# folbricht/desync

Hardware: AMD Instinct MI355X
Metric: GiB/s chunked (device-resident blob→cut list), 16/64/256KiB, 1/2/4/8 MI355X (higher is better)
Workload: dtype u8; 1 GPU; 32 GiB uniform blob per GPU (BASELINE config 5 shard shape), desync make min/avg/max 16/64/256 KiB, device-resident blob -> cut list in HBM; bytes_per_gpu=34359738368, chunks=524384, parallelism=single GPU, jobs_in_flight=4

## Files before the change

### desync_amd/_lib.py

```python
from __future__ import annotations

import ctypes
import os
import threading

HERE = os.path.dirname(os.path.abspath(__file__))
LIB_PATH = os.environ.get("DSX_LIB_PATH") or os.path.join(HERE, "libdsx.so")

DSX_OUT_HOST = 0
DSX_OUT_DEVICE = 1
DSX_NO_SYNC = 2
DSX_TIMED = 16
DSX_SEAM_MAX_CANDS = 1024
DSX_SEAM_MAX_CUTS = 1024

DSX_OK = 0
DSX_E_MIN_TOO_SMALL = -1
DSX_E_MIN_GT_MAX = -2
DSX_E_MIN_GT_AVG = -3
DSX_E_AVG_GT_MAX = -4
DSX_E_AVG_RANGE = -5
DSX_E_INVAL = -6
DSX_E_CAPACITY = -7
DSX_E_HIP = -8
DSX_E_NOMEM = -9
DSX_E_INTERRUPTED = -10
DSX_E_IO = -11
DSX_E_STATE = -12
DSX_E_INTERNAL = -13
DSX_E_RESYNC = -14
DSX_E_PEER = -15
DSX_STREAM_EOF = 1
DSX_STREAM_SYNC = 2
DSX_SEAM_DEVICE = 8
DSX_SEAM_LAST = 1
DSX_SEAM_REWALKED = 2
DSX_SEAM_ERROR = 4
DSX_SEAM_REDO = 16

EXPORTS = (
    "dsx_params_init", "dsx_strerror", "dsx_abi_version", "dsx_ctx_create", "dsx_ctx_destroy",
    "dsx_last_error", "dsx_cancel", "dsx_cut_device", "dsx_sync", "dsx_result", "dsx_cut_host",
    "dsx_cut_fd", "dsx_stream_begin", "dsx_stream_push", "dsx_stream_pop", "dsx_stream_advance",
    "dsx_stream_done", "dsx_stream_end", "dsx_stream_chunk_data", "dsx_stream_buffer",
    "dsx_stream_commit", "dsx_stream_flush", "dsx_stream_ids", "dsx_stream_chunk_id",
    "dsx_stream_pop_many", "dsx_stream_window", "dsx_stream_unpop", "dsx_shard_local", "dsx_shard_resolve",
    "dsx_selftest_boundary", "dsx_gen_uniform", "dsx_gen_dedup", "dsx_chunk_ids",
    "dsx_get_stats", "dsx_debug_trace", "dsx_index_fd", "dsx_index_host", "dsx_copy",
    "dsx_ids_fd", "dsx_ids_host", "dsx_progress", "dsx_shard_resolve_async", "dsx_shard_collect",
    "dsx_ctx_stream", "dsx_stamps_begin", "dsx_stamps_end", "dsx_host_copy",
    "dsx_host_sha512_256", "dsx_idset_create", "dsx_idset_destroy", "dsx_idset_count", "dsx_dedup",
)
DSX_DIGEST_SHA512_256 = 0
DSX_DIGEST_SHA256 = 1
DSX_ENDS_DEVICE = 4
DSX_HOST_SHA_SCALAR = 1
DSX_IDS_DEVICE = 32
DSX_SIZES = 64
DSX_POS_NONE = 0xFFFFFFFF


class Params(ctypes.Structure):

    _fields_ = [
        ("min", ctypes.c_uint64), ("avg", ctypes.c_uint64), ("max", ctypes.c_uint64),
        ("discriminator", ctypes.c_uint32), ("inverse_odd", ctypes.c_uint32),
        ("qmax", ctypes.c_uint32), ("qbias", ctypes.c_uint32), ("rot", ctypes.c_int32),
        ("reserved", ctypes.c_uint32),
    ]


class Stats(ctypes.Structure):
    _fields_ = [
        ("chunks", ctypes.c_uint64), ("candidates", ctypes.c_uint64), ("pieces", ctypes.c_uint64),
        ("repaired_segments", ctypes.c_uint64), ("dense_fallbacks", ctypes.c_uint64),
        ("scan_ms", ctypes.c_float), ("stitch_ms", ctypes.c_float),
        ("chunks_discarded", ctypes.c_uint64),
        ("device_bytes", ctypes.c_uint64),
        ("host_tail_chunks", ctypes.c_uint64),
    ]


class DedupTotals(ctypes.Structure):

    _fields_ = [(n, ctypes.c_uint64) for n in
                ("total", "unique", "in_seed", "size", "size_not_in_seed")]


class ScanStamp(ctypes.Structure):

    _fields_ = [(n, ctypes.c_uint64) for n in
                ("seq", "bytes", "t_first", "t_last", "wave_cycles", "wave_ticks", "waves", "reserved")]

    @property
    def ms(self):
        return (self.t_last - self.t_first) / 1e5

    @property
    def mhz(self):
        return 100.0 * self.wave_cycles / self.wave_ticks if self.wave_ticks else 0.0

    @property
    def busy(self):
        span = self.t_last - self.t_first
        return self.wave_ticks / (self.waves * span) if self.waves and span else 0.0


class Seam(ctypes.Structure):
    _fields_ = [
        ("shard_start", ctypes.c_uint64), ("shard_len", ctypes.c_uint64), ("total", ctypes.c_uint64),
        ("first_cand_beyond", ctypes.c_uint64), ("exit_cut", ctypes.c_uint64),
        ("window_end", ctypes.c_uint64), ("entry", ctypes.c_uint64),
        ("ncands", ctypes.c_uint32), ("ncuts", ctypes.c_uint32),
        ("flags", ctypes.c_uint32), ("pad", ctypes.c_uint32),
        ("cands", ctypes.c_uint64 * DSX_SEAM_MAX_CANDS),
        ("cuts", ctypes.c_uint64 * DSX_SEAM_MAX_CUTS),
    ]


_lib = None
_lock = threading.RLock()


def _share_torch_hip_runtime():
    try:
        import torch
    except ImportError:
        return
    path = os.path.join(os.path.dirname(torch.__file__), "lib", "libamdhip64.so")
    if os.path.exists(path):
        ctypes.CDLL(path, mode=ctypes.RTLD_GLOBAL)


PRODUCT_ENV = ("DSX_TAIL_SPLIT", "DSX_LANE_TARGET", "DSX_SEG_FLOOR", "DSX_SCAN_NT",
               "DSX_DIGEST_PC", "DSX_DIGEST_LPT", "DSX_INDEX_WINDOW", "DSX_INDEX_SLOT",
               "DSX_INDEX_READERS", "DSX_INDEX_HOST_TAIL", "DSX_HOST_THREADS")
DIAG_ENV = {"DSX_SCAN_VARIANT": "0", "DSX_SCAN_CFG": "0", "DSX_FUSE": "0", "DSX_TEST_MODE": None,
            "DSX_DIGEST_PC_CHUNKS": "2", "DSX_PREFETCH": "0", "DSX_REGIONS_PER_SLOT": "1",
            "DSX_SCAN_LINE": "1", "DSX_SCAN_TRACE": "0", "DSX_WAVE_MAJOR": "1",
            "DSX_FIXUP_FAST": "1", "DSX_FINISH": "1", "DSX_SEG_MAX": "4", "DSX_SEG_TARGET": "4096",
            "DSX_DIGEST_PF": "1", "DSX_TAIL_MULT": "1", "DSX_LANE_BYTES": None,
            "DSX_STITCH_CUS": "0", "DSX_SCAN_MASK": "0", "DSX_SCAN_PRIO": None,
            "DSX_STREAM_BATCH": None, "DSX_NOOP_BEFORE_SCAN": None, "DSX_WALK_WGS": "2",
            "DSX_WALK_NT": "576", "DSX_TAIL_LOG": None, "DSX_FEED_THREADS": None, "DSX_FEED_MULTI": None,
            "DSX_FEED_MID": None, "DSX_SIDE_PRIO": "1",
            "DSX_FEED_CUT_END": None, "DSX_SHARE_NS": "45", "DSX_SHARE_PC": "1", "DSX_SHARE_SLACK": "0", "DSX_CTX_PRIO": "1", "DSX_FEED_EXTRA": None, "DSX_SHARE_MULTI": "1", "DSX_FINE_TAIL": "33554432", "DSX_FINE_DIV": "4"}


def lib():
    global _lib
    with _lock:
        if _lib is not None:
            return _lib
        if not os.path.exists(LIB_PATH):
            raise ImportError(
                f"{LIB_PATH} is missing: build it with __graft_entry__.build() "
                "(make -C desync_amd/csrc). desync_amd has no CPU fallback.")
        diag_env = [k for k, dflt in DIAG_ENV.items() if os.environ.get(k, "") not in ("", dflt)]
        if diag_env and not os.path.basename(LIB_PATH).startswith("libdsx_diag"):
            raise ImportError(
                f"{', '.join(diag_env)} selects a diagnostic path (scan ablations, other "
                "geometries, rejected experiments), which only the diagnostic build reads: "
                "make -C desync_amd/csrc diag and set "
                "DSX_LIB_PATH=desync_amd/libdsx_diag.so")
        _share_torch_hip_runtime()
        L = ctypes.CDLL(LIB_PATH)
        u64, u32, i32, vp = ctypes.c_uint64, ctypes.c_uint32, ctypes.c_int, ctypes.c_void_p
        P = ctypes.POINTER
        sig = {
            "dsx_params_init": (i32, [u64, u64, u64, P(Params)]),
            "dsx_strerror": (ctypes.c_char_p, [i32]),
            "dsx_abi_version": (i32, []),
            "dsx_ctx_create": (i32, [i32, P(vp)]),
            "dsx_ctx_destroy": (i32, [vp]),
            "dsx_last_error": (ctypes.c_char_p, [vp]),
            "dsx_cancel": (i32, [vp]),
            "dsx_progress": (i32, [vp, P(u64)]),
            "dsx_cut_device": (i32, [vp, vp, u64, P(Params), vp, u64, P(u64), u32]),
            "dsx_sync": (i32, [vp]),
            "dsx_result": (i32, [vp, P(u64)]),
            "dsx_cut_host": (i32, [vp, vp, u64, P(Params), vp, u64, P(u64)]),
            "dsx_cut_fd": (i32, [vp, i32, u64, u64, P(Params), vp, u64, P(u64)]),
            "dsx_stream_begin": (i32, [vp, P(Params)]),
            "dsx_stream_push": (i32, [vp, vp, u64, i32]),
            "dsx_stream_pop": (i32, [vp, P(u64), P(u64)]),
            "dsx_stream_advance": (i32, [vp, u64]),
            "dsx_stream_done": (i32, [vp]),
            "dsx_stream_end": (i32, [vp]),
            "dsx_stream_buffer": (i32, [vp, u64, P(vp)]),
            "dsx_stream_commit": (i32, [vp, u64, i32]),
            "dsx_stream_flush": (i32, [vp, P(u64), P(u64)]),
            "dsx_stream_ids": (i32, [vp, i32]),
            "dsx_stream_chunk_id": (vp, [vp]),
            "dsx_stream_pop_many": (i32, [vp, vp, vp, u64, P(u64), P(u64)]),
            "dsx_stream_window": (i32, [vp, P(vp), P(u64), P(u64)]),
            "dsx_stream_unpop": (i32, [vp, u64]),
            "dsx_stream_chunk_data": (vp, [vp]),
            "dsx_shard_local": (i32, [vp, vp, u64, u64, u64, u64, P(Params), vp, u32]),
            "dsx_shard_resolve": (i32, [vp, vp, i32, i32, vp, vp, u64, P(u64), u32]),
            "dsx_shard_resolve_async": (i32, [vp, vp, i32, i32, vp, u64, vp]),
            "dsx_shard_collect": (i32, [vp, vp, vp, P(ctypes.c_int32), P(u64)]),
            "dsx_ctx_stream": (i32, [vp, P(vp)]),
            "dsx_selftest_boundary": (i32, [vp, P(Params), i32, u64, u64, P(u64)]),
            "dsx_gen_uniform": (i32, [vp, vp, u64, u64, u64]),
            "dsx_gen_dedup": (i32, [vp, vp, u64, u64, u64, ctypes.c_double]),
            "dsx_chunk_ids": (i32, [vp, vp, u64, u64, vp, u64, vp, u32, i32]),
            "dsx_get_stats": (i32, [vp, P(Stats)]),
            "dsx_copy": (i32, [vp, vp, vp, u64]),
            "dsx_index_fd": (i32, [vp, i32, u64, u64, P(Params), i32, vp, vp, u64, P(u64)]),
            "dsx_index_host": (i32, [vp, vp, u64, P(Params), i32, vp, vp, u64, P(u64)]),
            "dsx_debug_trace": (i32, [vp, vp, u64, P(u64), P(u64)]),
            "dsx_ids_fd": (i32, [vp, i32, u64, u64, u64, vp, u64, i32, vp]),
            "dsx_ids_host": (i32, [vp, vp, u64, u64, vp, u64, i32, vp]),
            "dsx_stamps_begin": (i32, [vp, u64]),
            "dsx_stamps_end": (i32, [vp, vp, u64, P(u64)]),
            "dsx_host_copy": (i32, [vp, vp, u64, i32]),
            "dsx_host_sha512_256": (i32, [vp, vp, u64, vp, i32, i32]),
            "dsx_idset_create": (i32, [vp, vp, u64, u32, P(vp)]),
            "dsx_idset_destroy": (i32, [vp, vp]),
            "dsx_idset_count": (i32, [vp, P(u64), P(u64)]),
            "dsx_dedup": (i32, [vp, vp, vp, u64, u64, vp, vp, vp, P(DedupTotals), u32]),
        }
        for name, (res, args) in sig.items():
            f = getattr(L, name)
            f.restype = res
            f.argtypes = args
        _lib = L
        return L


class DsxError(RuntimeError):
    def __init__(self, code, detail=""):
        self.code = code
        msg = lib().dsx_strerror(code).decode()
        super().__init__(f"{msg}" + (f": {detail}" if detail else ""))


def check(rc, ctx=None):
    if rc < 0:
        detail = ""
        if ctx is not None and rc in (DSX_E_HIP, DSX_E_INTERNAL, DSX_E_NOMEM):
            d = lib().dsx_last_error(ctx)
            detail = d.decode() if d else ""
        raise DsxError(rc, detail)
    return rc


class Context:

    def __init__(self, device=0):
        h = ctypes.c_void_p()
        rc = lib().dsx_ctx_create(int(device), ctypes.byref(h))
        if rc != DSX_OK:
            why = lib().dsx_last_error(None)
            raise DsxError(rc, f"cannot create a dsx context on HIP device {device}"
                           + (f" ({why.decode()})" if why else ""))
        self.h = h
        self.device = device

    def close(self):
        if self.h:
            lib().dsx_ctx_destroy(self.h)
            self.h = None

    def __del__(self):
        try:
            self.close()
        except Exception:
            pass

    def stats(self):
        s = Stats()
        check(lib().dsx_get_stats(self.h, ctypes.byref(s)), self.h)
        return s

    def stamps_begin(self, max_launches):
        check(lib().dsx_stamps_begin(self.h, int(max_launches)), self.h)
        self._stamp_cap = int(max_launches)

    def stamps_end(self):
        cap = getattr(self, "_stamp_cap", 0)
        buf = (ScanStamp * max(1, cap))()
        n = ctypes.c_uint64()
        check(lib().dsx_stamps_end(self.h, buf, cap, ctypes.byref(n)), self.h)
        return list(buf[:min(cap, n.value)])


_default = {}
_pool = {}


def default_context(device=0):
    ctx = _default.get(device)
    if ctx is None:
        ctx = Context(device)
        _default[device] = ctx
    return ctx


_POOL_IDLE = 4


def _env_key(device):
    return (device, tuple(sorted((k, v) for k, v in os.environ.items() if k.startswith("DSX_"))))


def acquire_context(device=0):
    key = _env_key(device)
    ctx = None
    with _lock:
        stale = [c for k in list(_pool) if k[0] == device and k != key for c in _pool.pop(k)]
        idle = _pool.setdefault(key, [])
        while idle and ctx is None:
            ctx = idle.pop()
            ctx = ctx if ctx.h else None
    for c in stale:
        c.close()
    if ctx is None:
        ctx = Context(device)
        ctx._pool_key = key
    return ctx


def release_context(ctx):
    if ctx is None or not ctx.h:
        return
    key = getattr(ctx, "_pool_key", None) or _env_key(ctx.device)
    with _lock:
        idle = _pool.setdefault(key, [])
        if len(idle) < _POOL_IDLE:
            idle.append(ctx)
            return
    ctx.close()


class pooled_context:

    def __init__(self, device=0):
        self.device = device
        self.ctx = None

    def __enter__(self):
        self.ctx = acquire_context(self.device)
        return self.ctx

    def __exit__(self, *exc):
        release_context(self.ctx)
        self.ctx = None
        return False


def reset_context_pool():
    with _lock:
        idle = [c for cs in _pool.values() for c in cs]
        _pool.clear()
    for c in idle:
        c.close()
```

### desync_amd/csrc/dsx_api.cpp

```cpp
#include <hip/hip_runtime.h>
#include <unistd.h>

#include <algorithm>
#include <atomic>
#include <cerrno>
#include <cmath>
#include <cstdarg>
#include <cstdio>
#include <cstdlib>
#include <cstring>
#include <deque>
#include <string>
#include <vector>

#include "dsx_engine.h"

using namespace dsx;

static_assert(sizeof(dsx_seam_t) == 7 * 8 + 4 * 4 + 8 * (DSX_SEAM_MAX_CANDS + DSX_SEAM_MAX_CUTS),
              "dsx_seam_t layout");

static void release_kept(dsx_ctx* c);


int set_hip_err(dsx_ctx* c, hipError_t e, const char* what) {
  char buf[256];
  snprintf(buf, sizeof buf, "%s: %s", what, hipGetErrorString(e));
  c->err = buf;
  return e == hipErrorOutOfMemory || e == hipErrorMemoryAllocation ? DSX_E_NOMEM : DSX_E_HIP;
}

static uint32_t discriminator_from_avg(uint64_t avg) {
  volatile double a = (double)avg;
  volatile double den = -1.42888852e-7 * a;
  den = den + 1.33237515;
  volatile double q = a / den;
  if (!(q >= 1.0 && q < 4294967296.0)) return 0u;
  return (uint32_t)q;
}

static uint32_t mod_inverse32(uint32_t d) {
  uint32_t x = d;
  for (int i = 0; i < 5; ++i) x *= 2u - d * x;
  return x;
}

extern "C" int dsx_abi_version(void) { return DSX_ABI_VERSION; }

extern "C" int dsx_params_init(uint64_t min, uint64_t avg, uint64_t max, dsx_params_t* out) {
  if (!out) return DSX_E_INVAL;
  if (min < 48) return DSX_E_MIN_TOO_SMALL;
  if (min > max) return DSX_E_MIN_GT_MAX;
  if (min > avg) return DSX_E_MIN_GT_AVG;
  if (avg > max) return DSX_E_AVG_GT_MAX;
  const uint32_t d = discriminator_from_avg(avg);
  if (d == 0) return DSX_E_AVG_RANGE;
  const uint32_t k = (uint32_t)__builtin_ctz(d);
  const uint32_t odd = d >> k;
  memset(out, 0, sizeof *out);
  out->min = min;
  out->avg = avg;
  out->max = max;
  out->discriminator = d;
  out->inverse_odd = mod_inverse32(odd);
  out->qbias = odd > 1u ? 1u : 0u;
  out->qmax = 0xFFFFFFFFu / d - out->qbias;
  out->rot = (int32_t)k;
  return DSX_OK;
}

extern "C" const char* dsx_strerror(int code) {
  switch (code) {
    case DSX_OK: return "ok";
    case DSX_E_MIN_TOO_SMALL: return "min chunk size too small, must be over 48";
    case DSX_E_MIN_GT_MAX: return "min chunk size must not be greater than max";
    case DSX_E_MIN_GT_AVG: return "min chunk size must not be greater than avg";
    case DSX_E_AVG_GT_MAX: return "avg chunk size must not be greater than max";
    case DSX_E_AVG_RANGE: return "avg chunk size out of range for discriminatorFromAvg";
    case DSX_E_INVAL: return "invalid argument";
    case DSX_E_CAPACITY: return "output capacity too small";
    case DSX_E_HIP: return "HIP runtime error";
    case DSX_E_NOMEM: return "out of memory";
    case DSX_E_INTERRUPTED: return "interrupted";
    case DSX_E_IO: return "I/O error";
    case DSX_E_STATE: return "invalid stream state";
    case DSX_E_INTERNAL: return "internal error";
    case DSX_E_RESYNC: return "seam records changed: all-gather them again and resolve again";
    case DSX_E_PEER: return "another rank failed (its seam record carries DSX_SEAM_ERROR)";
    default: return "unknown error";
  }
}

static TestConsts make_tc(const dsx_params_t* p) {
  TestConsts tc;
  tc.d = p->discriminator;
  tc.dm1 = p->discriminator - 1u;
  tc.inv = p->inverse_odd;
  tc.qmax = p->qmax;
  tc.qbias = p->qbias;
  tc.rot = (uint32_t)p->rot;
  tc.rcp = 1.0f / (float)p->discriminator;
  tc.c0 = 12582911.0f;
  tc.madc = p->discriminator - 1u - (p->discriminator << 22);
  const uint32_t k = (uint32_t)p->rot;
  tc.tadd = p->inverse_odd - 1u;
  tc.vmax = (uint32_t)(((1ull << 32) / p->discriminator) << k);
  tc.dodd = p->discriminator >> k;
  tc.ninv = 0u - p->inverse_odd;
  tc.vmax1 = tc.vmax + 1u;
  return tc;
}

static int pick_mode(const dsx_ctx* c, uint32_t d) {
  if (c->force_mode >= 0 && c->force_mode <= 2) {
    if (c->force_mode != 2 || (d & (d - 1u)) != 0) return c->force_mode;
  }
  if ((d & (d - 1u)) != 0) return 2;
  return (d > 1024u && d < (1u << 22)) ? 1 : 0;
}

static char g_create_err[256];

extern "C" int dsx_ctx_create(int device, dsx_ctx_t** out) {
  if (!out) return DSX_E_INVAL;
  *out = nullptr;
  g_create_err[0] = 0;
  dsx_ctx* c = new dsx_ctx();
  c->device = device;
#define CREATE_STEP(expr)                                                              \
  do {                                                                                 \
    hipError_t e_ = (expr);                                                            \
    if (e_ != hipSuccess) {                                                            \
      snprintf(g_create_err, sizeof g_create_err, "%s: %s (%d)", #expr,                \
               hipGetErrorString(e_), (int)e_);                                        \
      dsx_ctx_destroy(c);                                                              \
      return e_ == hipErrorOutOfMemory ? DSX_E_NOMEM : DSX_E_HIP;                      \
    }                                                                                  \
  } while (0)
  CREATE_STEP(hipSetDevice(device));
  hipDeviceProp_t prop;
  CREATE_STEP(hipGetDeviceProperties(&prop, device));
  c->ncu = prop.multiProcessorCount;
  if (const char* v = getenv("DSX_TAIL_SPLIT")) c->tail_split = std::max(0, std::min(8, atoi(v)));
  if (const char* v = getenv("DSX_LANE_TARGET"))
    c->lane_target = (uint32_t)std::max(384, std::min((int)kLineLaneMax, atoi(v)));
  if (const char* v = getenv("DSX_SEG_FLOOR")) c->seg_floor = (uint64_t)std::max(0L, atol(v));
  if (const char* v = getenv("DSX_SCAN_NT")) c->scan_nt = atoi(v) & 3;
  if (const char* v = getenv("DSX_DIGEST_PC")) c->digest_pc = atoi(v);
  if (const char* v = getenv("DSX_DIGEST_LPT")) c->digest_lpt = atoi(v) != 0;
  if (const char* v = getenv("DSX_INDEX_WINDOW")) c->index_window = (uint64_t)std::max(1L << 16, atol(v));
  if (const char* v = getenv("DSX_INDEX_SLOT")) c->index_slot = (uint64_t)std::max(1L << 12, atol(v));
  if (const char* v = getenv("DSX_INDEX_READERS")) c->index_readers = std::max(1, std::min(32, atoi(v)));
  if (const char* v = getenv("DSX_INDEX_HOST_TAIL")) c->index_host_tail = std::max(-1L, atol(v));
#if DSX_DIAG
  if (const char* m = getenv("DSX_TEST_MODE")) c->force_mode = atoi(m);
  if (const char* v = getenv("DSX_SCAN_VARIANT")) c->variant = atoi(v);
  if (const char* v = getenv("DSX_SCAN_CFG")) c->scan_cfg = std::min(5, std::max(0, atoi(v)));
  if (const char* v = getenv("DSX_DIGEST_PC_CHUNKS")) c->digest_pc_chunks = std::max(1, atoi(v));
  if (const char* v = getenv("DSX_PREFETCH")) c->prefetch_batches = std::max(0, atoi(v));
  if (const char* v = getenv("DSX_REGIONS_PER_SLOT")) c->regions_per_slot = std::max(1, atoi(v));
  if (const char* v = getenv("DSX_SCAN_LINE")) c->scan_line = atoi(v) != 0;
  if (const char* v = getenv("DSX_SCAN_TRACE")) {
    c->scan_trace = atoi(v) != 0;
    c->trace_keep = atoi(v) == 2;
  }
  if (const char* v = getenv("DSX_WAVE_MAJOR")) c->wave_major = atoi(v) != 0;
  if (const char* v = getenv("DSX_FIXUP_FAST")) c->fixup_fast = atoi(v) != 0;
  if (const char* v = getenv("DSX_FINISH")) c->finish = atoi(v) != 0;
  if (const char* v = getenv("DSX_FUSE")) c->fuse = atoi(v) != 0;
  if (const char* v = getenv("DSX_SEG_MAX")) c->seg_max_mult = std::max(1, atoi(v));
  if (const char* v = getenv("DSX_SEG_TARGET")) c->seg_target = (uint64_t)std::max(0L, atol(v));
  if (const char* v = getenv("DSX_WALK_WGS")) c->walk_wgs = std::max(1, std::min(4, atoi(v)));
  if (const char* v = getenv("DSX_WALK_NT")) c->walk_nt = atoi(v) == 576 ? 576 : 256;
  if (const char* v = getenv("DSX_DIGEST_PF")) c->digest_pf = atoi(v) != 0;
  if (const char* v = getenv("DSX_TAIL_MULT")) c->tail_mult = std::max(1, std::min(4, atoi(v)));
  if (const char* v = getenv("DSX_LANE_BYTES")) {
    const long lb = atol(v);
    if (lb >= 48 && lb % 48 == 0 && lb <= (long)kMaxLaneBytes) c->lane_bytes_override = (uint32_t)lb;
  }
  if (const char* v = getenv("DSX_STITCH_CUS")) c->stitch_cus = std::max(0, std::min(c->ncu / 2, atoi(v)));
  if (const char* v = getenv("DSX_SCAN_MASK")) c->scan_mask = atoi(v) != 0;
#endif
  {
    int least = 0, greatest = 0;
    CREATE_STEP(hipDeviceGetStreamPriorityRange(&least, &greatest));
#if DSX_DIAG
    if (const char* v = getenv("DSX_CTX_PRIO"))
      if (atoi(v) == 0) greatest = 0;
#endif
    CREATE_STEP(hipStreamCreateWithPriority(&c->stream, hipStreamNonBlocking, greatest));
    CREATE_STEP(hipStreamCreateWithPriority(&c->copy_stream, hipStreamNonBlocking, greatest));
  }
  c->scan_stream = c->stream;
#if DSX_DIAG
  if (c->stitch_cus > 0) {
    hipStream_t ss = nullptr;
    if (c->scan_mask) {
      std::vector<uint32_t> mask((c->ncu + 31) / 32, 0u);
      for (int i = 0; i < c->ncu - c->stitch_cus; ++i) mask[i / 32] |= 1u << (i % 32);
      CREATE_STEP(hipExtStreamCreateWithCUMask(&ss, (uint32_t)mask.size(), mask.data()));
    } else {
      int least = 0, greatest = 0;
      CREATE_STEP(hipDeviceGetStreamPriorityRange(&least, &greatest));
      const char* pv = getenv("DSX_SCAN_PRIO");
      CREATE_STEP(hipStreamCreateWithPriority(&ss, hipStreamNonBlocking,
                                              pv && atoi(pv) == 0 ? least : greatest));
    }
    c->scan_stream = ss;
    for (int i = 0; i < 2; ++i) {
      CREATE_STEP(hipEventCreateWithFlags(&c->ev_scan[i], hipEventDisableTiming));
      CREATE_STEP(hipEventCreateWithFlags(&c->ev_stitch[i], hipEventDisableTiming));
    }
  }
#endif
  CREATE_STEP(hipHostMalloc((void**)&c->h_state, sizeof(HostState), hipHostMallocCoherent));
  CREATE_STEP(hipHostMalloc((void**)&c->h_ring, kQueueDepth * sizeof(HostState), hipHostMallocCoherent));
  memset(c->h_ring, 0, kQueueDepth * sizeof(HostState));
  c->h_cur = c->h_state;
  for (uint32_t i = 0; i < kQueueDepth; ++i)
    CREATE_STEP(hipEventCreateWithFlags(&c->q_ev[i], hipEventDisableTiming));
  CREATE_STEP(hipHostMalloc((void**)&c->h_res, 4 * sizeof(uint64_t)));
#if DSX_DIAG
  CREATE_STEP(hipHostMalloc((void**)&c->h_tasks, dsx_ctx::kTaskRing * sizeof(TaskArgs), hipHostMallocCoherent));
#endif
  memset(c->h_state, 0, sizeof(HostState));
  CREATE_STEP(c->state.ensure(1));
  CREATE_STEP(c->overflow.ensure(kQueueWords));
  CREATE_STEP(hipMemset(c->overflow.p, 0, kQueueWords * sizeof(uint32_t)));
  CREATE_STEP(hipMemset(c->state.p, 0, sizeof(DevState)));
#undef CREATE_STEP
  *out = c;
  return DSX_OK;
}

extern "C" int dsx_ctx_destroy(dsx_ctx_t* c) {
  if (!c) return DSX_OK;
  (void)hipSetDevice(c->device);
  if (c->stream) (void)hipStreamSynchronize(c->stream);
  if (c->copy_stream) (void)hipStreamSynchronize(c->copy_stream);
  if (c->scan_stream && c->scan_stream != c->stream) (void)hipStreamSynchronize(c->scan_stream);
  c->region_cnt.release(); c->region_list.release(); c->overflow.release(); c->rep_cnt.release(); c->rep_from.release();
  c->region_cnt2.release(); c->region_list2.release();
  c->flag_list.release(); c->lane_slot.release(); c->seg_info.release(); c->stage.release();
  c->dg_ends.release(); c->dg_ids.release(); c->dg_queue.release();
  c->dg_order.release(); c->dg_cls.release();
  c->rep.release(); c->out_off.release(); c->out.release(); c->state.release();
  c->seg_info2.release(); c->stage2.release(); c->spec.release(); c->spec2.release();
  release_kept(c);
  c->zero_word.release();
  c->d_seam.release(); c->d_all.release(); c->d_ext.release(); c->d_info.release(); c->d_emit.release();
  if (c->h_res) (void)hipHostFree(c->h_res);
  if (c->h_tasks) (void)hipHostFree(c->h_tasks);
  index_release(c);
  stream_release(c);
  idset_release(c);
  if (c->h_state) (void)hipHostFree(c->h_state);
  if (c->h_ring) (void)hipHostFree(c->h_ring);
  for (uint32_t i = 0; i < kQueueDepth; ++i)
    if (c->q_ev[i]) (void)hipEventDestroy(c->q_ev[i]);
  for (hipEvent_t e : c->pev) (void)hipEventDestroy(e);
  for (auto& v : c->q_pev)
    for (hipEvent_t e : v) (void)hipEventDestroy(e);
  for (int i = 0; i < 2; ++i) {
    if (c->ev_scan[i]) (void)hipEventDestroy(c->ev_scan[i]);
    if (c->ev_stitch[i]) (void)hipEventDestroy(c->ev_stitch[i]);
  }
  if (c->scan_stream && c->scan_stream != c->stream) (void)hipStreamDestroy(c->scan_stream);
  if (c->stream) (void)hipStreamDestroy(c->stream);
  if (c->copy_stream) (void)hipStreamDestroy(c->copy_stream);
  delete c;
  return DSX_OK;
}

extern "C" const char* dsx_last_error(dsx_ctx_t* c) { return c ? c->err.c_str() : g_create_err; }

extern "C" int dsx_cancel(dsx_ctx_t* c) {
  if (!c) return DSX_E_INVAL;
  c->cancel.store(1);
  return DSX_OK;
}

extern "C" int dsx_progress(dsx_ctx_t* c, uint64_t* bytes) {
  if (!c || !bytes) return DSX_E_INVAL;
  uint64_t v = c->prog_done.load();
  if (c->prog_active.load()) {
    const uint64_t cur = ((volatile HostState*)c->h_state)->carry;
    if (cur > v && cur <= c->prog_len.load()) {
      uint64_t seen = v;
      while (seen < cur && !c->prog_done.compare_exchange_weak(seen, cur)) {
      }
      v = seen > cur ? seen : cur;
    }
  }
  *bytes = v;
  return DSX_OK;
}

extern "C" int dsx_debug_trace(dsx_ctx_t* c, uint64_t* out, uint64_t cap, uint64_t* n_scan,
                               uint64_t* n_walk) {
  DSX_FLUSH_BEHIND(c);
  if (!c || !n_scan || !n_walk) return DSX_E_INVAL;
  *n_scan = c->trace_n;
  *n_walk = c->trace_walk_n;
  const uint64_t words = c->trace_keep ? 4 * (kScanTraceWords * c->trace_n + 10 * 65536ull)
                                       : kScanTraceWords * c->trace_n + 10 * c->trace_walk_n;
  if (!words || !out) return DSX_OK;
  HIPCHK(c, hipSetDevice(c->device));
  HIPCHK(c, hipStreamSynchronize(c->stream));
  const uint64_t k = std::min<uint64_t>(cap, words);
  HIPCHK(c, hipMemcpy(out, c->trace.p, k * sizeof(uint64_t), hipMemcpyDeviceToHost));
  return DSX_OK;
}

extern "C" int dsx_copy(dsx_ctx_t* c, void* dst, const void* src, uint64_t n) {
  DSX_FLUSH_BEHIND(c);
  if (!c || (n && (!dst || !src))) return DSX_E_INVAL;
  if (!n) return DSX_OK;
  HIPCHK(c, hipSetDevice(c->device));
  HIPCHK(c, hipStreamSynchronize(c->stream));
  HIPCHK(c, hipMemcpy(dst, src, n, hipMemcpyDefault));
  return DSX_OK;
}

static uint64_t ctx_device_bytes(const dsx_ctx* c) {
  uint64_t b = 0;
  auto add = [&](const auto& d) { b += d.n * sizeof(*d.p); };
  add(c->trace);
  add(c->region_cnt), add(c->region_list), add(c->overflow), add(c->rep_cnt), add(c->rep_from);
  add(c->flag_list), add(c->region_cnt2), add(c->region_list2), add(c->lane_slot);
  add(c->seg_info), add(c->stage), add(c->rep), add(c->out_off), add(c->out);
  add(c->dg_ends), add(c->dg_ids), add(c->dg_queue), add(c->dg_order), add(c->dg_cls);
  add(c->state), add(c->seg_info2), add(c->stage2), add(c->spec), add(c->spec2);
  for (int i = 0; i < dsx_ctx::Stream::kSlots; ++i)
    add(c->st.dbuf[i]), add(c->st.dout[i]), add(c->st.dids[i]);
  add(c->st.rng), add(c->st.dq);
  for (const auto& k : c->sh.kept) add(k.cnt), add(k.list);
  add(c->d_seam), add(c->d_all), add(c->zero_word), add(c->d_ext), add(c->d_info), add(c->d_emit);
  add(c->stamp_ring), add(c->idx_win[0]), add(c->idx_win[1]), add(c->idx_snap);
  return b + idset_device_bytes(c);
}

extern "C" int dsx_get_stats(dsx_ctx_t* c, dsx_stats_t* out) {
  if (!c || !out) return DSX_E_INVAL;
  *out = c->stats;
  out->device_bytes = ctx_device_bytes(c);
  return DSX_OK;
}

extern "C" int dsx_stamps_begin(dsx_ctx_t* c, uint64_t max_launches) {
  if (!c || max_launches == 0 || max_launches > 65536) return DSX_E_INVAL;
  HIPCHK(c, hipSetDevice(c->device));
  HIPCHK(c, hipStreamSynchronize(c->stream));
  if (c->scan_stream != c->stream) HIPCHK(c, hipStreamSynchronize(c->scan_stream));
  c->stamp_slots = (uint64_t)c->ncu * (uint64_t)c->scanl_waves;
  const uint64_t words = max_launches * c->stamp_slots * kStampWords;
  HIPCHK(c, grow(c, c->stamp_ring, words));
  HIPCHK(c, hipMemset(c->stamp_ring.p, 0, words * sizeof(uint64_t)));
  c->stamp_meta.clear();
  c->stamp_cap = max_launches;
  c->stamping = true;
  return DSX_OK;
}

extern "C" int dsx_stamps_end(dsx_ctx_t* c, dsx_scan_stamp_t* out, uint64_t cap, uint64_t* n) {
  if (!c || !n || (cap && !out)) return DSX_E_INVAL;
  const bool was = c->stamping;
  c->stamping = false;
  *n = 0;
  if (!was) return DSX_E_STATE;
  HIPCHK(c, hipSetDevice(c->device));
  HIPCHK(c, hipStreamSynchronize(c->stream));
  if (c->scan_stream != c->stream) HIPCHK(c, hipStreamSynchronize(c->scan_stream));
  const uint64_t k = c->stamp_meta.size();
  *n = k;
  const uint64_t m = std::min(cap, k);
  if (!m) return DSX_OK;
  const uint64_t per = c->stamp_slots * kStampWords;
  std::vector<uint64_t> raw(m * per);
  HIPCHK(c, hipMemcpy(raw.data(), c->stamp_ring.p, raw.size() * sizeof(uint64_t), hipMemcpyDeviceToHost));
  for (uint64_t i = 0; i < m; ++i) {
    dsx_scan_stamp_t s{};
    s.seq = c->stamp_meta[i].first;
    s.bytes = c->stamp_meta[i].second;
    s.t_first = ~0ull;
    for (uint64_t w = 0; w < c->stamp_slots; ++w) {
      const uint64_t* r = &raw[i * per + w * kStampWords];
      if (r[1] == 0) continue;
      s.t_first = std::min(s.t_first, r[0]);
      s.t_last = std::max(s.t_last, r[1]);
      s.wave_ticks += r[1] - r[0];
      s.wave_cycles += r[3] - r[2];
      ++s.waves;
    }
    if (!s.waves) s.t_first = 0;
    out[i] = s;
  }
  return DSX_OK;
}


static uint64_t stitch_seg(const dsx_ctx* c, const dsx_params_t* p, uint64_t n) {
  uint64_t seg = std::max<uint64_t>(c->seg_max_mult * p->max, c->seg_floor);
  if (c->seg_target)
    while ((n + seg - 1) / seg > c->seg_target + 1 && seg < (1ull << 26)) seg <<= 1;
  return seg;
}

int reset_state(dsx_ctx* c, uint64_t carry) {
  c->npiece_call = 0;
  c->init_pending = true;
  c->init_carry = carry;
  return DSX_OK;
}

int read_state(dsx_ctx* c, HostState* out) {
  HIPCHK(c, hipStreamSynchronize(c->stream));
  memcpy(out, (const void*)c->h_state, sizeof(HostState));
  if (out->seq != c->piece_seq) {
    c->err = "stale chain state (no piece completed)";
    return DSX_E_INTERNAL;
  }
  return DSX_OK;
}

int enqueue_piece(dsx_ctx* c, const CallCfg& cc, const uint8_t* d_piece, uint64_t halo,
                         uint64_t P, uint64_t len, bool is_last) {
  const dsx_params_t* p = cc.p;
  static const int kCfgWaves[6] = {8, 12, 16, 12, 8, 16};
  static const int kCfgBR[6] = {2, 1, 1, 2, 2, 2};
  const uint32_t delta = (uint32_t)((uintptr_t)d_piece & (kLine - 1));
  const bool line = c->scan_line && !cc.dense && P >= delta;
  const int W = line ? c->scanl_waves : kCfgWaves[c->scan_cfg];
  const int cfgBR = kCfgBR[c->scan_cfg];
  const bool split = c->scan_stream != c->stream;
  const int ncu_scan = c->ncu - (split ? c->stitch_cus : 0);
  const uint64_t slots_total = (uint64_t)ncu_scan * W;
  const uint64_t span = line ? len + delta : len;
  uint32_t S, LS;
  uint32_t batches;
  if (cc.dense) {
    S = kDenseS;
    LS = S;
  } else if (line) {
    const uint64_t lanes_min = slots_total * 64 * (uint64_t)c->regions_per_slot;
    const uint64_t per_lane = (span + lanes_min - 1) / lanes_min;
    const uint64_t rounds_needed = (per_lane + kLineLaneMax - 1) / kLineLaneMax;
    const uint64_t s = (span + rounds_needed * lanes_min - 1) / (rounds_needed * lanes_min);
    uint64_t m = (s + 3 * kLine - 1) / (3 * kLine);
    const uint64_t mcap = c->lane_target / (3 * kLine);
    if (m > mcap + mcap / 4 || rounds_needed > 1) m = std::min<uint64_t>(m, mcap);
    m = std::max<uint64_t>(1, std::min<uint64_t>(m, kLineLaneMax / (3 * kLine)));
    S = (uint32_t)(3 * kLine * m);
    if (c->lane_bytes_override && c->lane_bytes_override % (3 * kLine) == 0 &&
        c->lane_bytes_override <= kLineLaneMax)
      S = c->lane_bytes_override;
    LS = kLaneSlots;
  } else {
    const uint64_t lanes_min = slots_total * 64 * (uint64_t)c->regions_per_slot;
    const uint64_t per_lane = (len + lanes_min - 1) / lanes_min;
    const uint64_t rounds_needed = (per_lane + kMaxLaneBytes - 1) / kMaxLaneBytes;
    uint64_t s = (len + rounds_needed * lanes_min - 1) / (rounds_needed * lanes_min);
    const uint64_t BR = (uint64_t)cfgBR;
    uint64_t kb = (s / kRound + 1 + BR - 1) / BR;
    if (kb < 4) kb = 4;
    while (kRound * (BR * kb - 1) > kMaxLaneBytes) --kb;
    s = (uint64_t)kRound * (BR * kb - 1);
    if (c->lane_bytes_override && (c->lane_bytes_override / kRound + 1) % BR == 0)
      s = c->lane_bytes_override;
    S = (uint32_t)s;
    LS = kLaneSlots;
  }
  batches = line ? S / (3 * kLine) : (S / kRound + 1) / (uint32_t)cfgBR;
  const uint64_t region_bytes = 64ull * S;
  uint64_t nregions = len == 0 ? 0 : (span + region_bytes - 1) / region_bytes;
  uint64_t nbig = nregions, S2 = 0;
  if (line && !cc.dense && !cc.behind && c->tail_split > 1 && len > 0) {
    const uint64_t m = S / (3 * kLine), m2 = std::max<uint64_t>(1, m / (uint64_t)c->tail_split);
    const uint64_t tail = slots_total * region_bytes * (uint64_t)c->tail_mult;
    if (m2 < m && span >= 3 * tail) {
      const uint64_t rb2 = 64ull * 3 * kLine * m2;
      nbig = (span - tail) / region_bytes;
      nregions = nbig + (span - nbig * region_bytes + rb2 - 1) / rb2;
      S2 = 3 * kLine * m2;
    }
  }
  const uint64_t nlanes = nregions * 64;
  uint32_t rcap;
  if (cc.dense) {
    rcap = 64u * S;
  } else {
    const double expct = (double)region_bytes / (double)p->discriminator;
    rcap = (uint32_t)std::min<double>(64.0 * S, 4.0 * expct + 64.0);
    rcap = (rcap + 63u) & ~63u;
  }
  c->last_region_bytes = region_bytes;
  c->last_nregions = (uint32_t)nregions;
  c->last_region_cap = rcap;
  c->last_nbig = (uint32_t)nbig;
  c->last_region_bytes2 = S2 ? 64ull * S2 : 0;
  HIPCHK(c, grow(c, c->lane_slot, nlanes * LS));
  uint32_t *rcnt, *rlist;
  KeptPiece* kp = nullptr;
  if (cc.keep) {
    if (c->sh.nkept == cc.keep->size()) cc.keep->emplace_back();
    kp = &(*cc.keep)[c->sh.nkept++];
    HIPCHK(c, grow(c, kp->cnt, nregions));
    HIPCHK(c, grow(c, kp->list, nregions * rcap));
    rcnt = kp->cnt.p;
    rlist = kp->list.p;
  } else {
    const bool second = (split || cc.behind) && (c->piece_seq + 1) % 2 == 1;
    auto& bc = second ? c->region_cnt2 : c->region_cnt;
    auto& bl = second ? c->region_list2 : c->region_list;
    HIPCHK(c, grow(c, bc, nregions));
    HIPCHK(c, grow(c, bl, nregions * rcap));
    rcnt = bc.p;
    rlist = bl.p;
  }
  c->last_rcnt = rcnt;
  c->last_rlist = rlist;
  dsx_ctx::Behind me;
  TaskArgs tb{};
#if DSX_DIAG
  if (cc.behind) {
    const bool second = (c->piece_seq + 1) % 2 == 1;
    const uint64_t seg = stitch_seg(c, p, len);
    const uint64_t nseg = (len + seg - 1) / seg;
    const uint32_t scap = (uint32_t)(seg / p->min + 3);
    auto& bs = second ? c->seg_info2 : c->seg_info;
    auto& bt = second ? c->stage2 : c->stage;
    auto& bp = second ? c->spec2 : c->spec;
    if (bs.n < nseg || bt.n < nseg * scap || bp.n < nseg * scap) {
      int rc = flush_behind(c);
      if (rc) return rc;
      HIPCHK(c, grow(c, bs, nseg));
      HIPCHK(c, grow(c, bt, nseg * scap));
      HIPCHK(c, grow(c, bp, nseg * scap));
    }
    const double exp_per_seg = (double)seg / (double)p->discriminator + 8.0;
    me.wseg = (uint32_t)std::max(1.0, std::min(32.0, std::floor(kTaskCand / (2.0 * exp_per_seg)) - 1.0));
    me.fseg = 32;
    me.nw = (uint32_t)((nseg + me.wseg - 1) / me.wseg);
    me.nf = (uint32_t)((nseg + me.fseg - 1) / me.fseg);
    me.w.min = p->min;
    me.w.max = p->max;
    me.w.L = len;
    me.w.seg = seg;
    me.w.nseg = (uint32_t)nseg;
    me.w.scap = scap;
    me.w.seg_info = bs.p;
    me.w.stage = bt.p;
    me.w.spec = bp.p;
    me.f.seg_info = bs.p;
    me.f.stage = bt.p;
    me.f.spec = bp.p;
    me.f.nseg = (uint32_t)nseg;
    me.f.scap = scap;
    me.f.out = cc.d_out;
    me.f.out_cap = cc.out_cap;
    me.f.host_state = c->h_cur;
    for (const auto& b : c->behind) {
      if (!b.walked) {
        tb.w = b.w;
        tb.nw = b.nw;
        tb.wseg = b.wseg;
      } else {
        tb.f = b.f;
        tb.nf = b.nf;
        tb.fseg = b.fseg;
      }
    }
  }
#endif
  const uint64_t seq = ++c->piece_seq;
  const int par = (int)(seq & 1);
  hipStream_t ss = c->scan_stream;

  ScanArgs sa{};
  sa.base = d_piece;
  sa.halo = halo;
  sa.piece_abs = P;
  sa.len = len;
  sa.lane_bytes = S;
  sa.batches = batches;
  sa.nregions = (uint32_t)nregions;
  if (S2) {
    sa.nbig = (uint32_t)nbig;
    sa.lane_bytes2 = (uint32_t)S2;
    sa.batches2 = (uint32_t)(S2 / (3 * kLine));
  }
  sa.region_cap = rcap;
  sa.tc = make_tc(p);
  sa.min_pos = cc.min_pos;
  sa.lane_slots = LS;
  sa.pf_batches = (uint32_t)c->prefetch_batches;
  sa.lane_slot = c->lane_slot.p;
  sa.region_cnt = rcnt;
  sa.region_list = rlist;
  sa.overflow = c->overflow.p + (seq % kQueueSlots);
  sa.overflow_next = c->overflow.p + ((seq + 1) % kQueueSlots);
  sa.queue = c->overflow.p + 32 + 256 * (seq % kQueueSlots);
  sa.queue_next = c->overflow.p + 32 + 256 * ((seq + 1) % kQueueSlots);
  sa.wave_major = c->wave_major ? (cc.behind ? 2u : 1u) : 0u;
  sa.nt_loads = (uint32_t)c->scan_nt;
  if (c->pub_host) {
    sa.pub_state = c->state.p;
    sa.pub_host = c->pub_host;
    sa.pub_seq = c->pub_seq;
    c->pub_host = nullptr;
  }
  tb.counter = sa.queue + 1;
  tb.farrive = sa.queue + 2;

#if DSX_DIAG
  if (cc.behind) {
    TaskArgs* slot = c->h_tasks + (c->fuse_seq++ % dsx_ctx::kTaskRing);
    *slot = tb;
    sa.tasks = slot;
  }
#endif
  if (line) {
    const uint64_t hmin = std::min<uint64_t>(halo, kRound);
    sa.delta = delta;
    sa.shift0 = halo >= (uint64_t)delta + kLine
                    ? 0u
                    : (uint32_t)(16 * (((uint64_t)kLine + delta - hmin) / 16));
  }
  c->last_grid_P = line ? P - delta : P;
  if (c->stamping && line && c->stamp_meta.size() < c->stamp_cap && W == c->scanl_waves) {
    sa.stamp = c->stamp_ring.p + c->stamp_slots * kStampWords * c->stamp_meta.size();
    c->stamp_meta.emplace_back(seq, len);
  }
  if (c->scan_trace && line) {
    c->trace_n = (uint64_t)c->ncu * W;
    const uint64_t slot_words = kScanTraceWords * c->trace_n + 10 * 65536ull;
    HIPCHK(c, grow(c, c->trace, (c->trace_keep ? 4 : 1) * slot_words));
    c->trace_base = c->trace_keep ? (seq % 4) * slot_words : 0;
    const uint64_t tw = cc.behind ? 6 * c->trace_n : 0;
    HIPCHK(c, hipMemsetAsync(c->trace.p + c->trace_base, 0, (kScanTraceWords * c->trace_n + tw) * sizeof(uint64_t), ss));
    sa.trace = c->trace.p + c->trace_base;
    if (cc.behind) c->trace_walk_n = (tw + 9) / 10;
  }
  const uint32_t pi = c->npiece_call++;
  while (c->pev.size() < 3 * (size_t)(pi + 1)) {
    hipEvent_t e;
    HIPCHK(c, hipEventCreate(&e));
    c->pev.push_back(e);
  }
  if (split) HIPCHK(c, hipStreamWaitEvent(ss, c->ev_stitch[par], 0));
  if (c->timing) HIPCHK(c, hipEventRecord(c->pev[3 * pi], ss));
#if DSX_DIAG
  if (getenv("DSX_NOOP_BEFORE_SCAN")) hipLaunchKernelGGL(noop_kernel, dim3(1), dim3(64), 0, ss);
#endif
  {
    const uint64_t need_wg = std::max<uint64_t>(1, (nregions + W - 1) / W);
    const uint32_t grid = cc.behind ? (uint32_t)ncu_scan
                                    : (uint32_t)std::min<uint64_t>(need_wg, (uint64_t)ncu_scan);
    const dim3 g(grid), b(W * kWave);
    const int mode = pick_mode(c, p->discriminator);
#if DSX_DIAG
#define DSX_ABLATE(K, ...)                                                                 \
  if (c->variant == 1) hipLaunchKernelGGL((K<2, 1, __VA_ARGS__>), g, b, 0, ss, sa); \
  else if (c->variant == 3) hipLaunchKernelGGL((K<2, 3, __VA_ARGS__>), g, b, 0, ss, sa); \
  else if (c->variant == 4) hipLaunchKernelGGL((K<2, 4, __VA_ARGS__>), g, b, 0, ss, sa); \
  else
#define DSX_LV(K, V, ...)                                                                  \
  do {                                                                                     \
    if (sa.lane_bytes2) hipLaunchKernelGGL((K<2, V, __VA_ARGS__, false, true>), g, b, 0, ss, sa); \
    else hipLaunchKernelGGL((K<2, V, __VA_ARGS__, false, false>), g, b, 0, ss, sa);      \
  } while (0)
#define DSX_ABLATEL(K, ...)                                                                \
  if (c->variant == 1) DSX_LV(K, 1, __VA_ARGS__);                                        \
  else if (c->variant == 3) DSX_LV(K, 3, __VA_ARGS__);                                   \
  else if (c->variant == 4) DSX_LV(K, 4, __VA_ARGS__);                                   \
  else if (c->variant == 7 && mode == 2) DSX_LV(K, 7, __VA_ARGS__);                      \
  else if (c->variant == 8 && mode == 2) DSX_LV(K, 8, __VA_ARGS__);                      \
  else if (c->variant == 9 && mode == 2) DSX_LV(K, 9, __VA_ARGS__);                      \
  else if (c->variant == 10 && mode == 2) DSX_LV(K, 10, __VA_ARGS__);                    \
  else
#else
#define DSX_ABLATE(K, ...)
#define DSX_ABLATEL(K, ...)
#endif
#define DSX_LAUNCH(BR, NB, WV, SUB, PF)                                                    \
  do {                                                                                     \
    DSX_ABLATE(scan_kernel, BR, NB, WV, SUB, PF)                                           \
    if (mode == 2)                                                                         \
      hipLaunchKernelGGL((scan_kernel<2, 0, BR, NB, WV, SUB, PF>), g, b, 0, ss, sa); \
    else if (mode == 1)                                                                    \
      hipLaunchKernelGGL((scan_kernel<1, 0, BR, NB, WV, SUB, PF>), g, b, 0, ss, sa); \
    else                                                                                   \
      hipLaunchKernelGGL((scan_kernel<0, 0, BR, NB, WV, SUB, PF>), g, b, 0, ss, sa); \
  } while (0)
#if DSX_DIAG
#define DSX_TRACE_VARIANTS(WV, SUB, D)                                                    \
  if (c->variant == 5) DSX_LV(scanl_kernel, 5, WV, SUB, D);                               \
  else if (c->variant == 6 && mode == 2) DSX_LV(scanl_kernel, 6, WV, SUB, D);             \
  else
#else
#define DSX_TRACE_VARIANTS(WV, SUB, D)
#endif
#define DSX_LAUNCHL(WV, SUB, D, FU, TW)                                                   \
  do {                                                                                    \
    if (mode == 2)                                                                        \
      hipLaunchKernelGGL((scanl_kernel<2, 0, WV, SUB, D, FU, TW>), g, b, 0, ss, sa);      \
    else if (mode == 1)                                                                   \
      hipLaunchKernelGGL((scanl_kernel<1, 0, WV, SUB, D, FU, TW>), g, b, 0, ss, sa);      \
    else                                                                                  \
      hipLaunchKernelGGL((scanl_kernel<0, 0, WV, SUB, D, FU, TW>), g, b, 0, ss, sa);      \
  } while (0)
#if DSX_DIAG
    if (line && cc.behind) {
      DSX_LAUNCHL(8, 8, 1, true, false);
    } else
#endif
    if (line) {
      DSX_ABLATEL(scanl_kernel, 8, 8, 1)
      DSX_TRACE_VARIANTS(8, 8, 1)
      if (sa.lane_bytes2) DSX_LAUNCHL(8, 8, 1, false, true);
      else DSX_LAUNCHL(8, 8, 1, false, false);
    } else {
#if DSX_DIAG
      switch (c->scan_cfg) {
        case 1: DSX_LAUNCH(1, 2, 12, 4, false); break;
        case 2: DSX_LAUNCH(1, 2, 16, 4, false); break;
        case 3: DSX_LAUNCH(2, 1, 12, 8, false); break;
        case 4: DSX_LAUNCH(2, 1, 8, 8, false); break;
        case 5: DSX_LAUNCH(2, 1, 16, 4, false); break;
        default:
          if (c->prefetch_batches > 0) DSX_LAUNCH(2, 2, 8, 8, true);
          else DSX_LAUNCH(2, 2, 8, 8, false);
      }
#else
      DSX_LAUNCH(2, 2, 8, 8, false);
#endif
    }
#undef DSX_LAUNCH
#undef DSX_LAUNCHL
#undef DSX_ABLATE
#undef DSX_ABLATEL
#ifdef DSX_LV
#undef DSX_LV
#endif
#undef DSX_TRACE_VARIANTS
    HIPCHK(c, hipGetLastError());
  }
  if (c->timing) HIPCHK(c, hipEventRecord(c->pev[3 * pi + 1], ss));
  if (split) {
    HIPCHK(c, hipEventRecord(c->ev_scan[par], ss));
    HIPCHK(c, hipStreamWaitEvent(c->stream, c->ev_scan[par], 0));
  }
  PieceCands pc{};
  pc.P = c->last_grid_P;
  pc.RB = region_bytes;
  pc.RB2 = c->last_region_bytes2;
  pc.nbig = c->last_nbig;
  pc.nregions = (uint32_t)nregions;
  pc.region_cap = rcap;
  pc.region_cnt = rcnt;
  pc.region_list = rlist;
  pc.overflow = sa.overflow;
  if (kp) {
    kp->pc = pc;
    kp->P = P;
    kp->len = len;
  }
#if DSX_DIAG
  if (cc.behind) {
    me.w.pc = pc;
    me.f.overflow = sa.overflow;
    me.f.seq = seq;
    me.seq = seq;
    std::deque<dsx_ctx::Behind> next;
    for (auto& b : c->behind)
      if (!b.walked) {
        b.walked = true;
        next.push_back(b);
      }
    next.push_back(me);
    c->behind.swap(next);
    c->init_pending = false;
    c->last_finish = false;
    if (c->timing) HIPCHK(c, hipEventRecord(c->pev[3 * pi + 2], c->stream));
    c->stats.pieces++;
    return DSX_OK;
  }
#endif
  int rc = launch_stitch(c, cc, pc, P, len, is_last, seq, line && c->scan_trace);
  if (rc) return rc;
  if (split) HIPCHK(c, hipEventRecord(c->ev_stitch[par], c->stream));
  if (c->timing) HIPCHK(c, hipEventRecord(c->pev[3 * pi + 2], c->stream));
  c->stats.pieces++;
  return DSX_OK;
}

static int launch_publish(dsx_ctx* c, const StitchArgs& ta) {
  c->last_finish = ta.host_state != nullptr;
  if (!ta.host_state) return DSX_OK;
  if (c->defer_publish) {
    c->pub_host = ta.host_state;
    c->pub_seq = ta.seq;
    return DSX_OK;
  }
  hipLaunchKernelGGL(publish_kernel, dim3(1), dim3(64), 0, c->stream, ta);
  HIPCHK(c, hipGetLastError());
  return DSX_OK;
}

int flush_publish(dsx_ctx* c) {
  if (!c->pub_host) return DSX_OK;
  StitchArgs ta{};
  ta.state = c->state.p;
  ta.host_state = c->pub_host;
  ta.seq = c->pub_seq;
  c->pub_host = nullptr;
  HIPCHK(c, hipSetDevice(c->device));
  hipLaunchKernelGGL(publish_kernel, dim3(1), dim3(64), 0, c->stream, ta);
  HIPCHK(c, hipGetLastError());
  return DSX_OK;
}

int launch_stitch(dsx_ctx* c, const CallCfg& cc, const PieceCands& pc, uint64_t P, uint64_t len,
                  bool is_last, uint64_t seq, bool trace) {
  const dsx_params_t* p = cc.p;
  const uint64_t region_bytes = pc.RB;
  StitchArgs ta{};
  ta.chain.min = p->min;
  ta.chain.max = p->max;
  ta.chain.L = cc.L;
  ta.chain.PE = P + len;
  ta.chain.is_last = is_last ? 1u : 0u;
  ta.pc = pc;
  const uint64_t anchor = (P > cc.origin + p->max) ? P - p->max : cc.origin;
  const uint64_t end = is_last ? cc.L : P + len;
  const uint64_t seg = stitch_seg(c, p, end > anchor ? end - anchor : 1);
  const uint64_t nseg = end > anchor ? (end - anchor + seg - 1) / seg : 1;
  ta.anchor = anchor;
  ta.seg = seg;
  ta.nseg = (uint32_t)nseg;
  const double exp_per_seg = (double)seg / (double)p->discriminator + 8.0;
  uint64_t spg = std::max<uint64_t>(2, nseg / ((uint64_t)c->walk_wgs * (uint64_t)c->ncu));
  const bool wide = c->scan_stream != c->stream;
  if (wide)
    spg = std::max<uint64_t>(spg, (nseg + 2ull * c->stitch_cus - 1) / (2ull * c->stitch_cus));
  spg = std::min<uint64_t>(spg, (uint64_t)((double)kWalkLdsCap / (2.0 * exp_per_seg)) - 1);
  const uint64_t rb_min = pc.RB2 ? std::min<uint64_t>(region_bytes, pc.RB2) : region_bytes;
  const uint64_t max_spg_reg = rb_min ? (4000ull * rb_min) / seg : kMaxSpg;
  spg = std::min<uint64_t>(spg, max_spg_reg > 2 ? max_spg_reg - 2 : 1);
  spg = std::max<uint64_t>(1, std::min<uint64_t>(spg, kMaxSpg));
  ta.spg = (uint32_t)spg;
  ta.lds_cap = kWalkLdsCap;
  ta.scap = (uint32_t)(seg / p->min + 3);
  HIPCHK(c, grow(c, c->seg_info, nseg));
  HIPCHK(c, grow(c, c->stage, nseg * ta.scap));
  HIPCHK(c, grow(c, c->rep, nseg * ta.scap));
  HIPCHK(c, grow(c, c->rep_cnt, nseg));
  HIPCHK(c, grow(c, c->rep_from, nseg));
  HIPCHK(c, grow(c, c->flag_list, nseg));
  HIPCHK(c, grow(c, c->out_off, nseg));
  ta.seg_info = c->seg_info.p;
  ta.stage = c->stage.p;
  ta.rep = c->rep.p;
  ta.rep_cnt = c->rep_cnt.p;
  ta.rep_from = c->rep_from.p;
  ta.flag_list = c->flag_list.p;
  ta.out_off = c->out_off.p;
  ta.out = cc.d_out;
  ta.out_cap = cc.out_cap;
  ta.state = c->state.p;
  ta.host_state = c->h_cur;
  ta.seq = seq;
  ta.init = c->init_pending ? 1u : 0u;
  ta.init_carry = c->init_carry;
  c->init_pending = false;
  c->last_finish = false;
  const uint32_t walk_grid = (uint32_t)((nseg + spg - 1) / spg);
  if (trace && walk_grid <= 65536) {
    ta.trace = c->trace.p + c->trace_base + kScanTraceWords * c->trace_n;
    c->trace_walk_n = walk_grid;
  }
  const size_t walk_lds = (size_t)kWalkLdsCap * 4 + (kMaxSpg + 1) * 8;
  if (wide)
    hipLaunchKernelGGL(walk_kernel<1024>, dim3(walk_grid), dim3(1024), walk_lds, c->stream, ta);
  else if (c->walk_nt == 576 && spg == 8)
    hipLaunchKernelGGL(walk_kernel<576>, dim3(walk_grid), dim3(576), walk_lds, c->stream, ta);
  else
    hipLaunchKernelGGL(walk_kernel<256>, dim3(walk_grid), dim3(256), walk_lds, c->stream, ta);
  HIPCHK(c, hipGetLastError());
  if (c->finish && nseg <= 2048) {
    const dim3 fg((uint32_t)((nseg + 15) / 16));
    if (nseg <= 256) hipLaunchKernelGGL(finish_kernel<1>, fg, dim3(256), 0, c->stream, ta);
    else if (nseg <= 512) hipLaunchKernelGGL(finish_kernel<2>, fg, dim3(256), 0, c->stream, ta);
    else if (nseg <= 1024) hipLaunchKernelGGL(finish_kernel<4>, fg, dim3(256), 0, c->stream, ta);
    else hipLaunchKernelGGL(finish_kernel<8>, fg, dim3(256), 0, c->stream, ta);
    HIPCHK(c, hipGetLastError());
    return launch_publish(c, ta);
  }
  if (c->fixup_fast && nseg <= 9 * 1024) {
    if (nseg <= 1024) hipLaunchKernelGGL(fixup_fast_kernel<1>, dim3(1), dim3(1024), 0, c->stream, ta);
    else if (nseg <= 2048) hipLaunchKernelGGL(fixup_fast_kernel<2>, dim3(1), dim3(1024), 0, c->stream, ta);
    else if (nseg <= 4096) hipLaunchKernelGGL(fixup_fast_kernel<4>, dim3(1), dim3(1024), 0, c->stream, ta);
    else if (nseg <= 5120) hipLaunchKernelGGL(fixup_fast_kernel<5>, dim3(1), dim3(1024), 0, c->stream, ta);
    else if (nseg <= 8192) hipLaunchKernelGGL(fixup_fast_kernel<8>, dim3(1), dim3(1024), 0, c->stream, ta);
    else hipLaunchKernelGGL(fixup_fast_kernel<9>, dim3(1), dim3(1024), 0, c->stream, ta);
  } else {
    hipLaunchKernelGGL(fixup_kernel, dim3(1), dim3(1024), 0, c->stream, ta);
  }
  HIPCHK(c, hipGetLastError());
  hipLaunchKernelGGL(gather_kernel, dim3((uint32_t)nseg), dim3(256), 0, c->stream, ta);
  HIPCHK(c, hipGetLastError());
  return launch_publish(c, ta);
}

static int run_device(dsx_ctx* c, const uint8_t* d_blob, uint64_t len, CallCfg cc) {
  HIPCHK(c, hipSetDevice(c->device));
  int rc = reset_state(c, cc.origin);
  if (rc) return rc;
  const uint64_t piece = cc.dense ? kDensePiece : kPieceMax;
  for (uint64_t off = 0; off < len; off += piece) {
    if (c->cancel.load()) return DSX_E_INTERRUPTED;
    const uint64_t n = std::min(piece, len - off);
    rc = enqueue_piece(c, cc, d_blob + off, off + cc.halo0, cc.origin + off, n, off + n == len);
    if (rc) return rc;
  }
  return DSX_OK;
}

int ensure_attr_walk(dsx_ctx* c) {
  static bool done = false;
  if (!done) {
    HIPCHK(c, hipFuncSetAttribute((const void*)walk_kernel<256>,
                                  hipFuncAttributeMaxDynamicSharedMemorySize,
                                  (int)(kWalkLdsCap * 4 + (kMaxSpg + 1) * 8)));
    HIPCHK(c, hipFuncSetAttribute((const void*)walk_kernel<576>,
                                  hipFuncAttributeMaxDynamicSharedMemorySize,
                                  (int)(kWalkLdsCap * 4 + (kMaxSpg + 1) * 8)));
    HIPCHK(c, hipFuncSetAttribute((const void*)walk_kernel<1024>,
                                  hipFuncAttributeMaxDynamicSharedMemorySize,
                                  (int)(kWalkLdsCap * 4 + (kMaxSpg + 1) * 8)));
    done = true;
  }
  return DSX_OK;
}

int flush_behind(dsx_ctx* c) {
  const int rc = flush_tasks(c);
  return rc ? rc : flush_publish(c);
}

int flush_tasks(dsx_ctx* c) {
  if (c->behind.empty()) return DSX_OK;
#if DSX_DIAG
  HIPCHK(c, hipSetDevice(c->device));
  while (!c->behind.empty()) {
    TaskArgs tb{};
    tb.farrive = c->overflow.p + kArriveWord + 1;
    for (const auto& b : c->behind) {
      if (!b.walked) {
        tb.w = b.w;
        tb.nw = b.nw;
        tb.wseg = b.wseg;
      } else {
        tb.f = b.f;
        tb.nf = b.nf;
        tb.fseg = b.fseg;
      }
    }
    const uint32_t n = tb.nw + tb.nf;
    if (n) {
      hipLaunchKernelGGL(stitch_task_kernel, dim3((n + 3) / 4), dim3(256), 0, c->stream, tb);
      HIPCHK(c, hipGetLastError());
    }
    std::deque<dsx_ctx::Behind> next;
    for (auto& b : c->behind)
      if (!b.walked) {
        b.walked = true;
        next.push_back(b);
      }
    c->behind.swap(next);
  }
#endif
  return DSX_OK;
}

static bool behind_ok(dsx_ctx* c, const void* d_blob, uint64_t len, const dsx_params_t* p) {
#if !DSX_DIAG
  return false;
#endif
  if (!c->fuse || !c->scan_line || c->stitch_cus > 0 || c->variant) return false;
  if (len == 0 || len > kPieceMax || ((uintptr_t)d_blob & (kLine - 1)) != 0) return false;
  const uint64_t seg = stitch_seg(c, p, len);
  const double exp_per_seg = (double)seg / (double)p->discriminator + 8.0;
  return 4.0 * exp_per_seg <= (double)kTaskCand;
}

static int finish_call(dsx_ctx* c, uint64_t* n_out, uint64_t cap, bool* dense_retry) {
  HostState s;
  int rc = read_state(c, &s);
  if (rc) return rc;
  *dense_retry = false;
  if (s.err & kErrDense) {
    *dense_retry = true;
    return DSX_OK;
  }
  c->stats.chunks = s.total;
  c->stats.repaired_segments = s.repaired;
  c->stats.chunks_discarded = s.discarded;
  float scan = 0, stitch = 0;
  for (uint32_t i = 0; i < c->npiece_call; ++i) {
    float a = 0, b = 0;
    (void)hipEventElapsedTime(&a, c->pev[3 * i], c->pev[3 * i + 1]);
    (void)hipEventElapsedTime(&b, c->pev[3 * i + 1], c->pev[3 * i + 2]);
    scan += a;
    stitch += b;
  }
  c->stats.scan_ms = scan;
  c->stats.stitch_ms = stitch;
  *n_out = s.total;
  if ((s.err & kErrCapacity) || s.total > cap) return DSX_E_CAPACITY;
  return DSX_OK;
}

extern "C" int dsx_sync(dsx_ctx_t* c) {
  if (!c) return DSX_E_INVAL;
  int rc = flush_behind(c);
  if (rc) return rc;
  HIPCHK(c, hipStreamSynchronize(c->stream));
  return DSX_OK;
}

extern "C" int dsx_cut_device(dsx_ctx_t* c, const void* d_blob, uint64_t len, const dsx_params_t* p,
                              uint64_t* out_ends, uint64_t cap, uint64_t* n_out, uint32_t flags);

extern "C" int dsx_result(dsx_ctx_t* c, uint64_t* n_out) {
  if (!c || !n_out) return DSX_E_INVAL;
  if (c->pend.empty()) return DSX_E_STATE;
  const dsx_ctx::Pending q = c->pend.front();
  c->pend.pop_front();
  HIPCHK(c, hipSetDevice(c->device));
  if (q.behind) {
    for (const auto& b : c->behind)
      if (b.seq == q.seq) {
        const int rc = flush_behind(c);
        if (rc) return rc;
        break;
      }
  }
  if (c->pub_host && c->pub_seq == q.seq) {
    const int rc = flush_publish(c);
    if (rc) return rc;
  }
  if (q.done) HIPCHK(c, hipEventSynchronize(q.done));
  {
    const volatile uint64_t* sp = &c->h_ring[q.slot].seq;
    for (uint32_t spins = 1; *sp != q.seq; ++spins) {
      if (spins % 4096u == 0) {
        const hipError_t e = hipStreamQuery(c->stream);
        if (e == hipSuccess) break;
        if (e != hipErrorNotReady) return set_hip_err(c, e, "hipStreamQuery");
      }
      __builtin_ia32_pause();
    }
    std::atomic_thread_fence(std::memory_order_acquire);
  }
  HostState s;
  memcpy(&s, (const void*)&c->h_ring[q.slot], sizeof(HostState));
  if (s.seq != q.seq) {
    c->err = "stale chain state (queued call did not complete)";
    return DSX_E_INTERNAL;
  }
  if (s.err & (kErrDense | kErrRedo)) {
    if (s.err & kErrDense) c->stats.dense_fallbacks++;
    dsx_params_t p = q.p;
    return dsx_cut_device(c, q.d_blob, q.len, &p, q.out, q.cap, n_out, DSX_OUT_DEVICE);
  }
  c->stats.chunks = s.total;
  c->stats.repaired_segments = s.repaired;
  c->stats.chunks_discarded = s.discarded;
  float scan = 0, stitch = 0;
  for (uint32_t i = 0; i < q.npiece; ++i) {
    float a = 0, b = 0;
    (void)hipEventElapsedTime(&a, c->q_pev[q.slot][3 * i], c->q_pev[q.slot][3 * i + 1]);
    (void)hipEventElapsedTime(&b, c->q_pev[q.slot][3 * i + 1], c->q_pev[q.slot][3 * i + 2]);
    scan += a;
    stitch += b;
  }
  c->stats.scan_ms = scan;
  c->stats.stitch_ms = q.behind ? 0.0f : stitch;
  *n_out = s.total;
  if ((s.err & kErrCapacity) || s.total > q.cap) return DSX_E_CAPACITY;
  return DSX_OK;
}

extern "C" int dsx_cut_device(dsx_ctx_t* c, const void* d_blob, uint64_t len, const dsx_params_t* p,
                              uint64_t* out_ends, uint64_t cap, uint64_t* n_out, uint32_t flags) {
  if (!c || !p || !n_out || (len && !d_blob) || (cap && !out_ends)) return DSX_E_INVAL;
  c->cancel.store(0);
  int rc = ensure_attr_walk(c);
  if (rc) return rc;
  *n_out = 0;
  if (len == 0) return DSX_OK;
  const bool dev_out = (flags & DSX_OUT_DEVICE) != 0;
  const uint64_t need = len / p->min + 2;
  const bool queued = (flags & DSX_NO_SYNC) && dev_out;
  const bool fuse = queued && behind_ok(c, d_blob, len, p);
  if (!fuse) {
    rc = flush_tasks(c);
    if (rc) return rc;
  }
  if (!queued) {
    rc = flush_publish(c);
    if (rc) return rc;
  }
  if (queued) {
    if (c->pend.size() >= kQueueDepth) {
      c->err = "too many queued DSX_NO_SYNC calls (collect them with dsx_result)";
      return DSX_E_STATE;
    }
    CallCfg cc{p, len, 0, kRound, out_ends, cap, false};
    cc.behind = fuse;
    dsx_ctx::Pending q;
    q.d_blob = d_blob;
    q.len = len;
    q.cap = cap;
    q.p = *p;
    q.out = out_ends;
    q.slot = c->q_next++ % kQueueDepth;
    q.done = c->q_ev[q.slot];
    c->h_cur = &c->h_ring[q.slot];
    const bool timed = (flags & DSX_TIMED) != 0;
    c->timing = timed;
    if (timed) std::swap(c->pev, c->q_pev[q.slot]);
    c->defer_publish = c->scan_stream == c->stream;
    rc = run_device(c, (const uint8_t*)d_blob, len, cc);
    c->defer_publish = false;
    if (timed) std::swap(c->pev, c->q_pev[q.slot]);
    q.npiece = timed ? c->npiece_call : 0u;
    c->timing = true;
    c->h_cur = c->h_state;
    if (rc) return rc;
    q.behind = fuse;
    if (fuse || (!timed && c->last_finish)) q.done = nullptr;
    else HIPCHK(c, hipEventRecord(q.done, c->stream));
    q.seq = c->piece_seq;
    c->pend.push_back(q);
    return DSX_OK;
  }
  for (int attempt = 0; attempt < 2; ++attempt) {
    CallCfg cc{p, len, 0, kRound, nullptr, 0, attempt == 1};
    if (dev_out) {
      cc.d_out = out_ends;
      cc.out_cap = cap;
    } else {
      HIPCHK(c, grow(c, c->out, need));
      cc.d_out = c->out.p;
      cc.out_cap = need;
    }
    rc = run_device(c, (const uint8_t*)d_blob, len, cc);
    if (rc) return rc;
    bool dense = false;
    rc = finish_call(c, n_out, dev_out ? cap : need, &dense);
    if (dense) {
      c->stats.dense_fallbacks++;
      continue;
    }
    if (rc) return rc;
    if (!dev_out && *n_out > cap) return DSX_E_CAPACITY;
    if (!dev_out && *n_out) {
      HIPCHK(c, hipMemcpy(out_ends, c->out.p, *n_out * sizeof(uint64_t), hipMemcpyDeviceToHost));
    }
    return DSX_OK;
  }
  c->err = "dense-candidate path overflowed";
  return DSX_E_INTERNAL;
}

extern "C" int dsx_gen_uniform(dsx_ctx_t* c, void* d_dst, uint64_t offset, uint64_t len,
                               uint64_t seed) {
  if (!c || (len && !d_dst)) return DSX_E_INVAL;
  HIPCHK(c, hipSetDevice(c->device));
  if (!len) return DSX_OK;
  const uint64_t threads = (len + 15) / 16;
  const uint32_t grid = (uint32_t)std::min<uint64_t>((threads + 255) / 256, 65536);
  hipLaunchKernelGGL(gen_uniform_kernel, dim3(grid), dim3(256), 0, c->stream, (uint8_t*)d_dst,
                     offset, len, seed);
  HIPCHK(c, hipGetLastError());
  HIPCHK(c, hipStreamSynchronize(c->stream));
  return DSX_OK;
}

extern "C" int dsx_gen_dedup(dsx_ctx_t* c, void* d_dst, uint64_t offset, uint64_t len,
                             uint64_t seed, double p_repeat) {
  if (!c || (len && !d_dst) || !(p_repeat >= 0.0 && p_repeat < 1.0)) return DSX_E_INVAL;
  HIPCHK(c, hipSetDevice(c->device));
  if (!len) return DSX_OK;
  const uint32_t thresh = (uint32_t)std::min(4294967295.0, p_repeat * 4294967296.0);
  const uint64_t threads = (len + 15) / 16;
  const uint32_t grid = (uint32_t)std::min<uint64_t>((threads + 255) / 256, 65536);
  hipLaunchKernelGGL(gen_dedup_kernel, dim3(grid), dim3(256), 0, c->stream, (uint8_t*)d_dst,
                     offset, len, seed, thresh);
  HIPCHK(c, hipGetLastError());
  HIPCHK(c, hipStreamSynchronize(c->stream));
  return DSX_OK;
}

int launch_digest(dsx_ctx* c, DigestArgs da, uint64_t max_n, int algo, hipStream_t stream,
                  uint32_t* queue, bool serial, uint32_t max_blocks, int pc) {
  const bool own = stream == nullptr || serial;
  if (!stream) stream = c->stream;
  if (!queue) {
    HIPCHK(c, c->dg_queue.ensure(1));
    queue = c->dg_queue.p;
  }
  const uint64_t pc_lanes = (uint64_t)c->ncu * 64u;
  if (c->digest_pc >= 0) pc = c->digest_pc > 0 ? 1 : 0;
  if (pc > 0 || (pc < 0 && max_n <= pc_lanes * (uint64_t)c->digest_pc_chunks)) {
    uint64_t blocks = std::max<uint64_t>(1, std::min<uint64_t>((max_n + 63) / 64, c->ncu));
    if (max_blocks) blocks = std::min<uint64_t>(blocks, max_blocks);
    HIPCHK(c, hipMemsetAsync(queue, 0, 4, stream));
    da.queue = queue;
    da.nfirst = (uint32_t)std::min<uint64_t>(da.n, blocks * 64u);
    if (algo == DSX_DIGEST_SHA512_256)
      hipLaunchKernelGGL(digest_pc_kernel<Sha512>, dim3((uint32_t)blocks), dim3(128), 0, stream, da);
    else
      hipLaunchKernelGGL(digest_pc_kernel<Sha256>, dim3((uint32_t)blocks), dim3(128), 0, stream, da);
    HIPCHK(c, hipGetLastError());
    return DSX_OK;
  }
  int per_cu = 0;
  const bool sha512 = algo == DSX_DIGEST_SHA512_256;
#if DSX_DIAG
  const bool pf = c->digest_pf != 0;
#else
  constexpr bool pf = true;
#endif
  const void* kern = sha512 ? (const void*)digest_kernel<Sha512, true>
                            : (const void*)digest_kernel<Sha256, true>;
#if DSX_DIAG
  if (!pf)
    kern = sha512 ? (const void*)digest_kernel<Sha512, false>
                  : (const void*)digest_kernel<Sha256, false>;
#endif
  HIPCHK(c, hipOccupancyMaxActiveBlocksPerMultiprocessor(&per_cu, kern, kDigestThreads, 0));
  if (per_cu < 1) per_cu = 1;
  uint64_t blocks = std::max<uint64_t>(
      1, std::min<uint64_t>((max_n + kDigestThreads - 1) / kDigestThreads,
                            (uint64_t)per_cu * (uint64_t)c->ncu));
  if (max_blocks) blocks = std::min<uint64_t>(blocks, max_blocks);
  HIPCHK(c, hipMemsetAsync(queue, 0, 4, stream));
  da.queue = queue;
  da.nfirst = (uint32_t)std::min<uint64_t>(da.n, blocks * kDigestThreads);
  if (own && c->digest_lpt && max_n >= 8u * kDigestThreads && max_n < (1ull << 32)) {
    HIPCHK(c, grow(c, c->dg_order, max_n));
    HIPCHK(c, c->dg_cls.ensure(2 * kSizeClasses));
    HIPCHK(c, hipMemsetAsync(c->dg_cls.p, 0, kSizeClasses * sizeof(uint32_t), stream));
    const dim3 tiles((uint32_t)((max_n + kOrderTile - 1) / kOrderTile));
    hipLaunchKernelGGL(digest_order_count_kernel, tiles, dim3(256), 0, stream, da, c->dg_cls.p);
    hipLaunchKernelGGL(digest_order_scan_kernel, dim3(1), dim3(kSizeClasses), 0, stream,
                       (const uint32_t*)c->dg_cls.p, c->dg_cls.p + kSizeClasses);
    hipLaunchKernelGGL(digest_order_scatter_kernel, tiles, dim3(256), 0, stream, da,
                       c->dg_cls.p + kSizeClasses, c->dg_order.p);
    HIPCHK(c, hipGetLastError());
    da.order = c->dg_order.p;
  }
  if (sha512 && pf)
    hipLaunchKernelGGL((digest_kernel<Sha512, true>), dim3((uint32_t)blocks), dim3(kDigestThreads),
                       0, stream, da);
  else if (pf)
    hipLaunchKernelGGL((digest_kernel<Sha256, true>), dim3((uint32_t)blocks), dim3(kDigestThreads),
                       0, stream, da);
#if DSX_DIAG
  else if (sha512)
    hipLaunchKernelGGL((digest_kernel<Sha512, false>), dim3((uint32_t)blocks), dim3(kDigestThreads),
                       0, stream, da);
  else
    hipLaunchKernelGGL((digest_kernel<Sha256, false>), dim3((uint32_t)blocks), dim3(kDigestThreads),
                       0, stream, da);
#endif
  HIPCHK(c, hipGetLastError());
  return DSX_OK;
}

extern "C" int dsx_chunk_ids(dsx_ctx_t* c, const void* d_blob, uint64_t len, uint64_t start,
                             const uint64_t* ends, uint64_t n, void* ids, uint32_t flags,
                             int algo) {
  DSX_FLUSH_BEHIND(c);
  if (!c || (n && (!d_blob || !ends || !ids)) || (algo != DSX_DIGEST_SHA512_256 &&
                                                   algo != DSX_DIGEST_SHA256))
    return DSX_E_INVAL;
  if ((flags & ~(DSX_OUT_DEVICE | DSX_ENDS_DEVICE)) != 0) return DSX_E_INVAL;
  if (n == 0) return DSX_OK;
  if (n > 0xFFFFFFF0ull) return DSX_E_INVAL;
  if (!(flags & DSX_ENDS_DEVICE)) {
    uint64_t prev = start;
    for (uint64_t i = 0; i < n; ++i) {
      if (ends[i] < prev || ends[i] > len) {
        c->err = "chunk ends must be non-decreasing, start <= ends[0], ends[n-1] <= len";
        return DSX_E_INVAL;
      }
      prev = ends[i];
    }
  }
  HIPCHK(c, hipSetDevice(c->device));
  c->err.clear();
  const uint64_t* d_ends = ends;
  if (!(flags & DSX_ENDS_DEVICE)) {
    HIPCHK(c, grow(c, c->dg_ends, n));
    HIPCHK(c, hipMemcpyAsync(c->dg_ends.p, ends, n * 8, hipMemcpyHostToDevice, c->stream));
    d_ends = c->dg_ends.p;
  }
  uint8_t* d_ids = (uint8_t*)ids;
  if (!(flags & DSX_OUT_DEVICE)) {
    HIPCHK(c, grow(c, c->dg_ids, n * 32));
    d_ids = c->dg_ids.p;
  }
  DigestArgs da{};
  da.blob = (const uint8_t*)d_blob;
  da.len = len;
  da.ends = d_ends;
  da.first_start = start;
  da.n = n;
  da.ids = d_ids;
  int rc = launch_digest(c, da, n, algo);
  if (rc) return rc;
  if (!(flags & DSX_OUT_DEVICE))
    HIPCHK(c, hipMemcpyAsync(ids, d_ids, n * 32, hipMemcpyDeviceToHost, c->stream));
  HIPCHK(c, hipStreamSynchronize(c->stream));
  return DSX_OK;
}

extern "C" int dsx_selftest_boundary(dsx_ctx_t* c, const dsx_params_t* p, int mode, uint64_t h0,
                                     uint64_t n, uint64_t* mismatches) {
  DSX_FLUSH_BEHIND(c);
  if (!c || !p || !mismatches) return DSX_E_INVAL;
  HIPCHK(c, hipSetDevice(c->device));
  if (mode < 0) mode = pick_mode(c, p->discriminator);
  const uint32_t d = p->discriminator;
  if (mode > 2 || (mode == 2 && (d & (d - 1u)) == 0)) return DSX_E_INVAL;
  DevBuf<unsigned long long> m;
  HIPCHK(c, m.ensure(1));
  HIPCHK(c, hipMemsetAsync(m.p, 0, 8, c->stream));
  hipLaunchKernelGGL(boundary_selftest_kernel, dim3(4096), dim3(256), 0, c->stream, make_tc(p),
                     mode, h0, n, m.p);
  HIPCHK(c, hipGetLastError());
  unsigned long long v = 0;
  HIPCHK(c, hipMemcpyAsync(&v, m.p, 8, hipMemcpyDeviceToHost, c->stream));
  HIPCHK(c, hipStreamSynchronize(c->stream));
  m.release();
  *mismatches = v;
  return DSX_OK;
}

static void release_kept(dsx_ctx* c) {
  for (auto& k : c->sh.kept) {
    k.cnt.release();
    k.list.release();
  }
  c->sh.kept.clear();
  c->sh.nkept = 0;
}

static int shard_run(dsx_ctx* c, uint64_t entry, uint32_t rec_flags, bool rewalk,
                     bool async = false) {
  auto& sh = c->sh;
  const dsx_params_t* p = &sh.p;
  const bool is_last = sh.start + sh.len == sh.total;
  const uint64_t need = sh.len / p->min + 4;
  const uint64_t wend0 = sh.start + std::min<uint64_t>(sh.len, 32 * p->max);
  HIPCHK(c, hipSetDevice(c->device));
  HIPCHK(c, grow(c, c->d_seam, 1));
  const bool stitch_only = rewalk && !sh.dense && sh.nkept > 0;
  for (int attempt = 0; attempt < 2; ++attempt) {
    if (c->cancel.load()) return DSX_E_INTERRUPTED;
    HIPCHK(c, grow(c, c->out, need));
    const bool dense = attempt == 1 || (rewalk && sh.dense);
    CallCfg cc{p, sh.total, entry, kRound, c->out.p, need, dense};
    cc.halo0 = sh.start > 0 ? sh.halo : 0;
    int rc = DSX_OK;
    if (stitch_only) {
      HIPCHK(c, c->zero_word.ensure(1));
      HIPCHK(c, hipMemsetAsync(c->zero_word.p, 0, 4, c->stream));
      hipLaunchKernelGGL(state_init_kernel, dim3(1), dim3(64), 0, c->stream, (DevState*)c->state.p,
                         entry);
      HIPCHK(c, hipGetLastError());
      c->npiece_call = 0;
      for (size_t i = 0; i < sh.nkept && !rc; ++i) {
        PieceCands pc = sh.kept[i].pc;
        pc.overflow = c->zero_word.p;
        rc = launch_stitch(c, cc, pc, sh.kept[i].P, sh.kept[i].len,
                           is_last && i + 1 == sh.nkept, ++c->piece_seq, false);
      }
      if (rc) return rc;
      hipLaunchKernelGGL(seam_cands_kernel, dim3(1), dim3(64), 0, c->stream, sh.kept[0].pc,
                         sh.start, wend0, c->d_seam.p);
      HIPCHK(c, hipGetLastError());
    } else {
      sh.nkept = 0;
      cc.keep = dense ? nullptr : &sh.kept;
      sh.dense = dense;
      rc = reset_state(c, entry);
      if (rc) return rc;
      const uint64_t piece = cc.dense ? kDensePiece : kPieceMax;
      for (uint64_t off = 0; off < sh.len; off += piece) {
        const uint64_t n = std::min(piece, sh.len - off);
        rc = enqueue_piece(c, cc, sh.d + off, off + cc.halo0, sh.start + off, n,
                           is_last && off + n == sh.len);
        if (rc) return rc;
        if (off == 0) {
          PieceCands pc{};
          pc.P = c->last_grid_P;
          pc.RB = c->last_region_bytes;
          pc.RB2 = c->last_region_bytes2;
          pc.nbig = c->last_nbig;
          pc.nregions = c->last_nregions;
          pc.region_cap = c->last_region_cap;
          pc.region_cnt = cc.keep ? sh.kept[0].cnt.p : c->last_rcnt;
          pc.region_list = cc.keep ? sh.kept[0].list.p : c->last_rlist;
          pc.overflow = nullptr;
          hipLaunchKernelGGL(seam_cands_kernel, dim3(1), dim3(64), 0, c->stream, pc, sh.start,
                             wend0, c->d_seam.p);
          HIPCHK(c, hipGetLastError());
        }
      }
    }
    hipLaunchKernelGGL(seam_finalize_kernel, dim3(1), dim3(1), 0, c->stream, c->d_seam.p,
                       (const uint64_t*)c->out.p, (const DevState*)c->state.p, sh.start, sh.len,
                       sh.total, wend0, entry, (is_last ? (uint32_t)DSX_SEAM_LAST : 0u) | rec_flags);
    HIPCHK(c, hipGetLastError());
    if (async) {
      sh.nspec = ~0ull;
      return DSX_OK;
    }
    HostState st;
    rc = read_state(c, &st);
    if (rc) return rc;
    if ((st.err & kErrDense) && !stitch_only) {
      c->stats.dense_fallbacks++;
      continue;
    }
    if (st.err) {
      c->err = "shard: stitch error";
      return DSX_E_INTERNAL;
    }
    sh.nspec = st.total;
    c->stats.chunks = st.total;
    return DSX_OK;
  }
  c->err = "dense-candidate path overflowed";
  return DSX_E_INTERNAL;
}

static int seam_out(dsx_ctx* c, dsx_seam_t* seam, bool dev, bool wait = true) {
  HIPCHK(c, hipMemcpyAsync(seam, c->d_seam.p, sizeof(dsx_seam_t),
                           dev ? hipMemcpyDeviceToDevice : hipMemcpyDeviceToHost, c->stream));
  if (wait || !dev) HIPCHK(c, hipStreamSynchronize(c->stream));
  return DSX_OK;
}

extern "C" int dsx_shard_local(dsx_ctx_t* c, const void* d_shard, uint64_t halo,
                               uint64_t shard_start, uint64_t shard_len, uint64_t total,
                               const dsx_params_t* p, dsx_seam_t* seam, uint32_t flags) {
  DSX_FLUSH_BEHIND(c);
  if (!c || !p || !seam || (shard_len && !d_shard) || shard_start + shard_len > total ||
      (flags & ~(DSX_SEAM_DEVICE | DSX_NO_SYNC)) != 0 ||
      ((flags & DSX_NO_SYNC) && !(flags & DSX_SEAM_DEVICE)))
    return DSX_E_INVAL;
  const bool async = (flags & DSX_NO_SYNC) != 0;
  if (shard_start > 0 && halo < kRound) return DSX_E_INVAL;
  c->cancel.store(0);
  int rc = ensure_attr_walk(c);
  if (rc) return rc;
  auto& sh = c->sh;
  sh.d = (const uint8_t*)d_shard;
  sh.halo = halo;
  sh.start = shard_start;
  sh.len = shard_len;
  sh.total = total;
  sh.p = *p;
  sh.nspec = 0;
  sh.valid = false;
  if (shard_len == 0) {
    dsx_seam_t z;
    memset(&z, 0, sizeof z);
    z.shard_start = z.exit_cut = z.window_end = z.entry = shard_start;
    z.total = total;
    z.first_cand_beyond = UINT64_MAX;
    z.flags = shard_start == total ? DSX_SEAM_LAST : 0u;
    HIPCHK(c, grow(c, c->d_seam, 1));
    HIPCHK(c, hipMemcpyAsync(c->d_seam.p, &z, sizeof z, hipMemcpyHostToDevice, c->stream));
    sh.valid = true;
    return seam_out(c, seam, (flags & DSX_SEAM_DEVICE) != 0);
  }
  rc = shard_run(c, shard_start, 0u, false, async);
  if (rc) return rc;
  sh.valid = true;
  return seam_out(c, seam, (flags & DSX_SEAM_DEVICE) != 0, !async);
}

static int shard_outcome(dsx_ctx* c, int rank, dsx_seam_t* my_seam, bool seam_dev, uint64_t cap,
                         uint64_t* n_out) {
  const uint64_t status = c->h_res[0], n = c->h_res[1], entry = c->h_res[2];
  *n_out = 0;
  if (status == ~0ull) {
    c->err = "shard: resolve did not publish its result";
    return DSX_E_INTERNAL;
  }
  if (status == kSeamPeerFailed) return DSX_E_PEER;
  if (status != 0) {
    const bool redo = status == kSeamRedo;
    const int failing = redo ? (int)entry : (int)(status - 1);
    if (failing == rank) {
      auto& sh = c->sh;
      int rc = redo ? shard_run(c, sh.start, 0u, false) : shard_run(c, entry, DSX_SEAM_REWALKED, true);
      if (rc) {
        const size_t off = offsetof(dsx_seam_t, flags);
        uint32_t fl = 0;
        const hipMemcpyKind d2h = seam_dev ? hipMemcpyDeviceToHost : hipMemcpyHostToHost;
        const hipMemcpyKind h2d = seam_dev ? hipMemcpyHostToDevice : hipMemcpyHostToHost;
        (void)hipStreamSynchronize(c->stream);
        if (hipMemcpy(&fl, (const uint8_t*)my_seam + off, 4, d2h) == hipSuccess) {
          fl |= DSX_SEAM_ERROR;
          (void)hipMemcpy((uint8_t*)my_seam + off, &fl, 4, h2d);
        }
        return rc;
      }
      if (redo)
        c->stats.dense_fallbacks++;
      else
        c->stats.repaired_segments++;
      rc = seam_out(c, my_seam, seam_dev);
      if (rc) return rc;
    }
    return DSX_E_RESYNC;
  }
  *n_out = n;
  if (n > cap) return DSX_E_CAPACITY;
  return DSX_OK;
}

extern "C" int dsx_shard_resolve(dsx_ctx_t* c, const dsx_seam_t* all, int nranks, int rank,
                                 dsx_seam_t* my_seam, uint64_t* out_ends, uint64_t cap,
                                 uint64_t* n_out, uint32_t flags) {
  DSX_FLUSH_BEHIND(c);
  if (!c || !all || nranks < 1 || rank < 0 || rank >= nranks || !n_out || !my_seam ||
      (cap && !out_ends) || (flags & ~(DSX_SEAM_DEVICE | DSX_OUT_DEVICE)) != 0)
    return DSX_E_INVAL;
  auto& sh = c->sh;
  if (!sh.valid) return DSX_E_STATE;
  HIPCHK(c, hipSetDevice(c->device));
  const bool seam_dev = (flags & DSX_SEAM_DEVICE) != 0, out_dev = (flags & DSX_OUT_DEVICE) != 0;
  const dsx_seam_t* d_all = all;
  if (!seam_dev) {
    HIPCHK(c, grow(c, c->d_all, (size_t)nranks));
    HIPCHK(c, hipMemcpyAsync(c->d_all.p, all, sizeof(dsx_seam_t) * nranks, hipMemcpyHostToDevice,
                             c->stream));
    d_all = c->d_all.p;
  }
  HIPCHK(c, grow(c, c->d_ext, DSX_SEAM_MAX_CUTS + 4));
  HIPCHK(c, grow(c, c->d_info, 8));
  hipLaunchKernelGGL(seam_resolve_kernel, dim3(1), dim3(64), 0, c->stream, d_all, nranks, rank,
                     sh.p.min, sh.p.max, c->d_ext.p, c->d_info.p);
  HIPCHK(c, hipGetLastError());
  const uint64_t most = (sh.nspec == ~0ull ? sh.len / sh.p.min + 4 : sh.nspec) + DSX_SEAM_MAX_CUTS;
  uint64_t* dst = out_ends;
  uint64_t dcap = cap;
  if (!out_dev) {
    HIPCHK(c, grow(c, c->d_emit, most));
    dst = c->d_emit.p;
    dcap = most;
  }
  const uint32_t blocks = (uint32_t)std::min<uint64_t>((most + 255) / 256, 4096);
  c->h_res[0] = ~0ull;
  hipLaunchKernelGGL(shard_emit_kernel, dim3(blocks), dim3(256), 0, c->stream,
                     (const uint64_t*)c->d_info.p, (const uint64_t*)c->d_ext.p,
                     (const uint64_t*)c->out.p, (const DevState*)c->state.p, dst, dcap,
                     (volatile uint64_t*)c->h_res, (int32_t*)nullptr);
  HIPCHK(c, hipGetLastError());
  HIPCHK(c, hipStreamSynchronize(c->stream));
  int rc = shard_outcome(c, rank, my_seam, seam_dev, cap, n_out);
  if (rc) return rc;
  const uint64_t n = *n_out;
  if (!out_dev && n)
    HIPCHK(c, hipMemcpy(out_ends, c->d_emit.p, n * sizeof(uint64_t), hipMemcpyDeviceToHost));
  return DSX_OK;
}

extern "C" int dsx_shard_resolve_async(dsx_ctx_t* c, const dsx_seam_t* all, int nranks, int rank,
                                       uint64_t* out_ends, uint64_t cap, int32_t* d_code) {
  DSX_FLUSH_BEHIND(c);
  if (!c || !all || nranks < 1 || rank < 0 || rank >= nranks || !out_ends || !d_code)
    return DSX_E_INVAL;
  auto& sh = c->sh;
  if (!sh.valid) return DSX_E_STATE;
  HIPCHK(c, hipSetDevice(c->device));
  HIPCHK(c, grow(c, c->d_ext, DSX_SEAM_MAX_CUTS + 4));
  HIPCHK(c, grow(c, c->d_info, 8));
  hipLaunchKernelGGL(seam_resolve_kernel, dim3(1), dim3(64), 0, c->stream, all, nranks, rank,
                     sh.p.min, sh.p.max, c->d_ext.p, c->d_info.p);
  HIPCHK(c, hipGetLastError());
  const uint64_t most = sh.len / sh.p.min + 4 + DSX_SEAM_MAX_CUTS;
  const uint32_t blocks = (uint32_t)std::min<uint64_t>((std::min(most, cap) + 255) / 256 + 1, 4096);
  c->h_res[0] = ~0ull;
  hipLaunchKernelGGL(shard_emit_kernel, dim3(blocks), dim3(256), 0, c->stream,
                     (const uint64_t*)c->d_info.p, (const uint64_t*)c->d_ext.p,
                     (const uint64_t*)c->out.p, (const DevState*)c->state.p, out_ends, cap,
                     (volatile uint64_t*)c->h_res, d_code);
  HIPCHK(c, hipGetLastError());
  sh.pend_rank = rank;
  sh.pend_cap = cap;
  sh.pending = true;
  return DSX_OK;
}

extern "C" int dsx_shard_collect(dsx_ctx_t* c, dsx_seam_t* my_seam, const int32_t* d_agreed,
                                 int32_t* agreed, uint64_t* n_out) {
  DSX_FLUSH_BEHIND(c);
  if (!c || !my_seam || !n_out || (d_agreed && !agreed)) return DSX_E_INVAL;
  auto& sh = c->sh;
  if (!sh.pending) return DSX_E_STATE;
  sh.pending = false;
  HIPCHK(c, hipSetDevice(c->device));
  int32_t* h_code = (int32_t*)(c->h_res + 3);
  if (d_agreed)
    HIPCHK(c, hipMemcpyAsync(h_code, d_agreed, sizeof(int32_t), hipMemcpyDeviceToHost, c->stream));
  HIPCHK(c, hipStreamSynchronize(c->stream));
  if (d_agreed) *agreed = *h_code;
  if (d_agreed && *h_code >= 2) {
    const uint64_t status = c->h_res[0], n = c->h_res[1];
    *n_out = 0;
    if (status == ~0ull) return DSX_E_INTERNAL;
    if (status == 0 && n > sh.pend_cap) {
      *n_out = n;
      return DSX_E_CAPACITY;
    }
    return DSX_E_PEER;
  }
  int rc = shard_outcome(c, sh.pend_rank, my_seam, true, sh.pend_cap, n_out);
  if (rc == DSX_OK) c->stats.chunks = *n_out;
  return rc;
}

extern "C" int dsx_ctx_stream(dsx_ctx_t* c, void** stream) {
  DSX_FLUSH_BEHIND(c);
  if (!c || !stream) return DSX_E_INVAL;
  *stream = (void*)c->stream;
  return DSX_OK;
}
```

### desync_amd/csrc/dsx_engine.h

```cpp
#pragma once
#include <hip/hip_runtime.h>

#include <array>
#include <atomic>
#include <deque>
#include <functional>
#include <string>
#include <vector>

#include "../../include/dsx.h"
#include "dsx_common.h"
#include "dsx_digest.h"
#include "dsx_stitch.h"

namespace dsx {
template <class H, bool PF>
__global__ void digest_kernel(DigestArgs a);
template <class H>
__global__ void digest_pc_kernel(DigestArgs a);
template <int MODE, int VARIANT, int BR, int NBUF, int W, int SUB, bool PF>
__global__ void scan_kernel(ScanArgs a);
template <int MODE, int VARIANT, int W, int SUB, int D, bool FUSE, bool TWO>
__global__ void scanl_kernel(ScanArgs a);
__global__ void stitch_task_kernel(TaskArgs b);
template <int NT>
__global__ void walk_kernel(StitchArgs a);
__global__ void fixup_kernel(StitchArgs a);
template <int PER>
__global__ void fixup_fast_kernel(StitchArgs a);
template <int PER>
__global__ void finish_kernel(StitchArgs a);
__global__ void gather_kernel(StitchArgs a);
__global__ void publish_kernel(StitchArgs a);
__global__ void noop_kernel();
__global__ void state_init_kernel(DevState* st, uint64_t carry);
__global__ void gen_uniform_kernel(uint8_t* dst, uint64_t offset, uint64_t len, uint64_t seed);
__global__ void gen_dedup_kernel(uint8_t* dst, uint64_t offset, uint64_t len, uint64_t seed,
                                 uint32_t p_thresh);
__global__ void boundary_selftest_kernel(TestConsts tc, int mode, uint64_t h0, uint64_t n,
                                         unsigned long long* mismatches);
__global__ void seam_cands_kernel(PieceCands pc, uint64_t lo, uint64_t wend, dsx_seam_t* seam);
__global__ void seam_finalize_kernel(dsx_seam_t* seam, const uint64_t* cuts, const DevState* st,
                                     uint64_t shard_start, uint64_t shard_len, uint64_t total,
                                     uint64_t wend0, uint64_t entry, uint32_t flags);
__global__ void seam_resolve_kernel(const dsx_seam_t* all, int nranks, int rank, uint64_t min,
                                    uint64_t max, uint64_t* ext, uint64_t* info);
__global__ void shard_emit_kernel(const uint64_t* info, const uint64_t* ext, const uint64_t* spec,
                                  const DevState* st, uint64_t* out, uint64_t cap,
                                  volatile uint64_t* res, int32_t* code);

}

using namespace dsx;

namespace dsx_host {

constexpr uint64_t kPieceMax = 8ull << 30;
constexpr uint64_t kStreamBatch = 16ull << 20;
constexpr uint32_t kQueueDepth = 8;
constexpr uint32_t kWalkLdsCap = 8192;
constexpr uint32_t kDenseS = 48 * 9;
constexpr uint64_t kDensePiece = 32ull << 20;

template <class T>
struct DevBuf {
  T* p = nullptr;
  size_t n = 0;
  hipError_t ensure(size_t want) {
    if (want <= n && p) return hipSuccess;
    if (p) (void)hipFree(p);
    p = nullptr;
    n = 0;
    size_t sz = want < 16 ? 16 : want;
    hipError_t e = hipMalloc((void**)&p, sz * sizeof(T));
    if (e == hipSuccess) n = sz;
    return e;
  }
  void release() {
    if (p) (void)hipFree(p);
    p = nullptr;
    n = 0;
  }
};

}
using namespace dsx_host;

#include "dsx_idset.h"

struct KeptPiece {
  DevBuf<uint32_t> cnt, list;
  PieceCands pc{};
  uint64_t P = 0, len = 0;
};

struct dsx_ctx {
  int device = 0;
  int ncu = 256;
  hipStream_t stream = nullptr, copy_stream = nullptr;
  hipStream_t scan_stream = nullptr;
  int stitch_cus = 0;
  bool scan_mask = false;
  hipEvent_t ev_scan[2] = {}, ev_stitch[2] = {};
  bool timing = true;
  std::atomic<int> cancel{0};
  std::atomic<uint64_t> prog_done{0};
  std::atomic<uint64_t> prog_len{0};
  std::atomic<int> prog_active{0};
  std::string err;
  int force_mode = -1;
  int variant = 0;
  uint32_t lane_bytes_override = 0;
  int prefetch_batches = 0;
  int regions_per_slot = 1;
  int scan_cfg = 0;
  bool scan_line = true;
  int digest_pc = -1;
  int digest_pc_chunks = 2;
  int scanl_waves = 8;
  uint32_t lane_target = 8448;
  int tail_split = 4;
  int tail_mult = 1;
  uint64_t seg_max_mult = 4;
  uint64_t seg_floor = 1ull << 20;
  uint64_t seg_target = 4096;
  int walk_wgs = 2;
  int walk_nt = 576;
  bool scan_trace = false;
  bool wave_major = true;
  int scan_nt = 1;
  bool finish = true;
  bool fixup_fast = true;
  DevBuf<uint64_t> trace;
  uint64_t trace_n = 0, trace_walk_n = 0;
  bool trace_keep = false;
  uint64_t trace_base = 0;
  uint64_t last_grid_P = 0;

  DevBuf<uint32_t> region_cnt, region_list, overflow, rep_cnt, rep_from, flag_list;
  DevBuf<uint32_t> region_cnt2, region_list2;
  const uint32_t* last_rcnt = nullptr;
  const uint32_t* last_rlist = nullptr;
  DevBuf<uint32_t> lane_slot;
  DevBuf<SegInfo> seg_info;
  DevBuf<uint64_t> stage, rep, out_off, out;
  DevBuf<uint64_t> dg_ends;
  DevBuf<uint8_t> dg_ids;
  DevBuf<uint32_t> dg_queue;
  DevBuf<uint32_t> dg_order;
  DevBuf<uint32_t> dg_cls;
  int digest_lpt = 1;
  int digest_pf = 1;
  DevBuf<DevState> state;
  HostState* h_state = nullptr;
  uint64_t piece_seq = 0;
  bool init_pending = false;
  uint64_t last_region_bytes = 0;
  uint32_t last_nregions = 0, last_region_cap = 0;
  uint32_t last_nbig = 0;
  uint64_t last_region_bytes2 = 0;
  uint64_t init_carry = 0;
  bool last_finish = false;
  bool defer_publish = false;
  HostState* pub_host = nullptr;
  uint64_t pub_seq = 0;
  struct Behind {
    WalkJob w;
    FinishJob f;
    uint32_t nw = 0, nf = 0, wseg = 1, fseg = 1;
    bool walked = false;
    uint64_t seq = 0;
  };
  std::deque<Behind> behind;
  bool fuse = false;
  static constexpr uint32_t kTaskRing = 16;
  TaskArgs* h_tasks = nullptr;
  uint64_t fuse_seq = 0;
  DevBuf<SegInfo> seg_info2;
  DevBuf<uint64_t> stage2;
  DevBuf<uint64_t> spec, spec2;

  struct Stream {
    static constexpr int kSlots = 3;
    struct Batch {
      uint64_t P, len, seq;
      bool last, ids;
      int slot;
    };
    bool active = false, eof = false, done = false, final_pending = false;
    bool fresh = true;
    bool dense = false;
    dsx_params_t p{};
    uint64_t batch = 32ull << 20;
    uint8_t* h = nullptr;
    uint64_t hcap = 0, hbase = 0, hend = 0;
    uint64_t cur = 0;
    uint64_t pin = 0;
    std::vector<uint64_t> grp;
    std::vector<std::array<uint8_t, 32>> grp_ids;
    uint64_t origin = 0;
    uint64_t sched = 0;
    uint64_t carry = 0;
    uint64_t fresh_carry = 0;
    uint64_t skip = 0;
    std::deque<uint64_t> cuts;
    std::deque<Batch> fly;
    int next_slot = 0;
    const uint8_t* last_chunk = nullptr;
    int ids = -1;
    std::deque<std::array<uint8_t, 32>> idq;
    uint8_t last_id[32] = {};
    bool has_id = false;
    hipStream_t dg_stream = nullptr;
    DevBuf<uint8_t> dbuf[kSlots];
    DevBuf<uint64_t> dout[kSlots];
    uint64_t* hcut[kSlots] = {};
    uint64_t hcut_cap[kSlots] = {};
    HostState* hstate = nullptr;
    hipEvent_t copy_ev[kSlots] = {}, done_ev[kSlots] = {}, stitch_ev[kSlots] = {};
    DevBuf<uint8_t> dids[kSlots];
    uint8_t* hids[kSlots] = {};
    uint64_t hids_cap[kSlots] = {};
    DevBuf<uint64_t> rng;
    DevBuf<uint32_t> dq;
  } st;

  struct Shard {
    const uint8_t* d = nullptr;
    uint64_t halo = 0, start = 0, len = 0, total = 0;
    dsx_params_t p{};
    uint64_t nspec = 0;
    bool pending = false;
    int pend_rank = 0;
    uint64_t pend_cap = 0;
    bool valid = false;
    bool dense = false;
    std::vector<KeptPiece> kept;
    size_t nkept = 0;
  } sh;
  DevBuf<dsx_seam_t> d_seam, d_all;
  DevBuf<uint32_t> zero_word;
  DevBuf<uint64_t> d_ext, d_info, d_emit;
  uint64_t* h_res = nullptr;

  dsx_stats_t stats{};
  DevBuf<uint64_t> stamp_ring;
  uint64_t stamp_slots = 0;
  bool stamping = false;
  uint64_t stamp_cap = 0;
  std::vector<std::pair<uint64_t, uint64_t>> stamp_meta;
  std::vector<hipEvent_t> pev;
  uint32_t npiece_call = 0;

  struct Pending {
    const void* d_blob = nullptr;
    uint64_t len = 0, cap = 0;
    dsx_params_t p{};
    uint64_t* out = nullptr;
    uint32_t slot = 0;
    uint64_t seq = 0;
    hipEvent_t done = nullptr;
    bool behind = false;
    uint32_t npiece = 0;
  };
  std::vector<hipEvent_t> q_pev[kQueueDepth];
  std::deque<Pending> pend;
  HostState* h_ring = nullptr;
  HostState* h_cur = nullptr;

  static constexpr int kIdxSlots = 8;
  uint64_t index_window = 1ull << 30;
  uint64_t index_slot = 32ull << 20;
  int index_readers = 4;
  int64_t index_host_tail = -1;
  uint8_t* idx_slots[kIdxSlots] = {};
  uint64_t idx_slot_bytes = 0;
  DevBuf<uint8_t> idx_win[2];
  DevBuf<uint64_t> idx_snap;
  hipEvent_t idx_copy_ev[kIdxSlots] = {};
  hipEvent_t idx_win_ev[2] = {};
  hipEvent_t idx_stitch_ev[2] = {};
  hipStream_t idx_dg_stream = nullptr;
  static constexpr int kIdxSide = 4;
  hipStream_t idx_side[kIdxSide] = {};
  DevBuf<uint32_t> idx_side_q;
  hipEvent_t q_ev[kQueueDepth] = {};
  uint32_t q_next = 0;

  IdsetScratch idset;
};

template <class T>
inline hipError_t grow(dsx_ctx* c, DevBuf<T>& b, size_t n) {
  if (b.p && b.n >= n) return hipSuccess;
  if (b.p) {
    (void)hipStreamSynchronize(c->stream);
    (void)hipStreamSynchronize(c->copy_stream);
    if (c->scan_stream != c->stream) (void)hipStreamSynchronize(c->scan_stream);
  }
  return b.ensure(n + n / 4 + 64);
}

inline hipError_t scan_wait(dsx_ctx* c, hipEvent_t ev) {
  return hipStreamWaitEvent(c->scan_stream, ev, 0);
}

int set_hip_err(dsx_ctx* c, hipError_t e, const char* what);

#define HIPCHK(ctx, expr)                                  \
  do {                                                     \
    hipError_t e_ = (expr);                                \
    if (e_ != hipSuccess) return set_hip_err(ctx, e_, #expr); \
  } while (0)

struct CallCfg {
  const dsx_params_t* p;
  uint64_t L;
  uint64_t origin;
  uint64_t min_pos;
  uint64_t* d_out;
  uint64_t out_cap;
  bool dense;
  uint64_t halo0 = 0;
  std::vector<KeptPiece>* keep = nullptr;
  bool behind = false;
};

int reset_state(dsx_ctx* c, uint64_t carry);
int read_state(dsx_ctx* c, HostState* out);
int enqueue_piece(dsx_ctx* c, const CallCfg& cc, const uint8_t* d_piece, uint64_t halo,
                  uint64_t P, uint64_t len, bool is_last);
int ensure_attr_walk(dsx_ctx* c);
void host_parallel(int parts, const std::function<void(int)>& fn);
int host_cpu_share();
hipError_t side_stream_create(hipStream_t* s);
bool host_sha_vec();
void host_sha512_256_one(const uint8_t* p, uint64_t n, uint8_t* out);
void host_sha512_256_x8(const uint8_t* const p[8], const uint64_t n[8], uint8_t* const out[8]);
int flush_behind(dsx_ctx* c);
int flush_tasks(dsx_ctx* c);
int flush_publish(dsx_ctx* c);
#define DSX_FLUSH_BEHIND(c)                  \
  do {                                       \
    if (c) {                                 \
      const int rc_fb_ = flush_behind(c);    \
      if (rc_fb_) return rc_fb_;             \
    }                                        \
  } while (0)
int launch_stitch(dsx_ctx* c, const CallCfg& cc, const PieceCands& pc, uint64_t P, uint64_t len,
                  bool is_last, uint64_t seq, bool trace);
int launch_digest(dsx_ctx* c, DigestArgs da, uint64_t max_n, int algo, hipStream_t stream = nullptr,
                  uint32_t* queue = nullptr, bool serial = false, uint32_t max_blocks = 0, int pc = -1);
void index_release(dsx_ctx* c);
void stream_release(dsx_ctx* c);
```

### desync_amd/csrc/dsx_stitch.h

```cpp
#pragma once
#include <stdint.h>

namespace dsx {

struct PieceCands {
  uint64_t P;
  uint64_t RB;
  uint32_t nregions;
  uint32_t region_cap;
  const uint32_t* region_cnt;
  const uint32_t* region_list;
  const uint32_t* overflow;
  uint64_t RB2;
  uint32_t nbig;
  uint32_t pad;
};

__host__ __device__ __forceinline__ uint64_t pc_region_base(const PieceCands& pc, uint64_t r) {
  return (pc.RB2 == 0 || r <= pc.nbig) ? r * pc.RB
                                       : (uint64_t)pc.nbig * pc.RB + (r - pc.nbig) * pc.RB2;
}
__host__ __device__ __forceinline__ uint64_t pc_region_of(const PieceCands& pc, uint64_t x) {
  const uint64_t big = (uint64_t)pc.nbig * pc.RB;
  return (pc.RB2 == 0 || x < big) ? x / pc.RB : pc.nbig + (x - big) / pc.RB2;
}

struct ChainParams {
  uint64_t min, max;
  uint64_t L;
  uint64_t PE;
  uint32_t is_last;
  uint32_t pad;
};

struct SegInfo {
  uint64_t E;
  uint64_t X;
  uint64_t Z;
  uint32_t cnt;
  uint32_t flags;
};
constexpr uint32_t kSegEnd = 1u;
constexpr uint32_t kSegUndet = 2u;
constexpr uint32_t kSegDense = 4u;
constexpr uint32_t kSegOverflow = 8u;

struct DevState {
  uint64_t carry;
  uint64_t total;
  uint64_t piece_cuts;
  uint64_t repaired;
  uint32_t done;
  uint32_t err;
  uint32_t active;
  uint32_t pad;
  uint64_t base;
  uint32_t skip;
  uint32_t pad2;
  uint64_t discarded;
};

struct HostState {
  uint64_t carry, total, repaired, discarded;
  uint32_t done, err;
  uint64_t seq;
};
constexpr uint32_t kErrCapacity = 1u;
constexpr uint32_t kErrDense = 2u;
constexpr uint32_t kErrRedo = 4u;

struct TaskSeg {
  uint64_t X, Z;
  uint32_t cnt, flags;
  uint32_t n2, f1;
};
struct WalkJob {
  PieceCands pc;
  uint64_t min, max, L;
  uint64_t seg;
  uint32_t nseg, scap;
  SegInfo* seg_info;
  uint64_t* stage;
  uint64_t* spec;
};
struct FinishJob {
  const SegInfo* seg_info;
  const uint64_t* stage;
  const uint64_t* spec;
  const uint32_t* overflow;
  uint32_t nseg, scap;
  uint64_t* out;
  uint64_t out_cap;
  HostState* host_state;
  uint64_t seq;
};
struct TaskArgs {
  WalkJob w;
  FinishJob f;
  uint32_t nw, nf;
  uint32_t wseg, fseg;
  uint32_t* counter;
  uint32_t* farrive;
};
constexpr uint32_t kTaskCand = 2048;
constexpr uint64_t kSeamPeerFailed = 0x7FFFFFFFFFFFFFFFull;
constexpr uint64_t kSeamRedo = 0x7FFFFFFFFFFFFFFEull;

constexpr uint32_t kMaxSpg = 255;

struct StitchArgs {
  ChainParams chain;
  PieceCands pc;
  uint64_t anchor;
  uint64_t seg;
  uint32_t nseg;
  uint32_t spg;
  uint32_t lds_cap;
  uint32_t scap;
  SegInfo* seg_info;
  uint64_t* stage;
  uint64_t* rep;
  uint32_t* rep_cnt;
  uint32_t* rep_from;
  uint32_t* flag_list;
  uint64_t* out_off;
  uint64_t* out;
  uint64_t out_cap;
  DevState* state;
  HostState* host_state;
  uint64_t seq;
  uint64_t* trace;
  uint64_t init_carry;
  uint32_t init;
  uint32_t pad_init;
};

}
```

### desync_amd/csrc/dsx_stitch.hip

```cpp
#include <hip/hip_runtime.h>

#include "dsx_chain.h"
#include "dsx_common.h"
#include "dsx_stitch.h"
#if DSX_DIAG
#include "dsx_tasks.h"
#endif

namespace dsx {

struct LdsSrc {
  const uint32_t* c;
  uint32_t n;
  uint32_t j;
  uint64_t lo;
  __device__ uint64_t first_in(uint64_t a, uint64_t b) {
    const uint64_t ar = a - lo;
    while (j < n && (uint64_t)c[j] <= ar) ++j;
    if (j < n) {
      const uint64_t p = lo + (uint32_t)__builtin_amdgcn_readfirstlane(c[j]);
      if (p <= b) return p;
    }
    return kNone;
  }
  __device__ void seek(uint64_t a) {
    const uint64_t ar = a < lo ? 0 : a - lo;
    uint32_t l = 0, h = n;
    while (l < h) {
      const uint32_t m = (l + h) >> 1;
      if ((uint64_t)c[m] <= ar) l = m + 1; else h = m;
    }
    j = l;
  }
};

struct GlobalSrc {
  const PieceCands* pc;
  __device__ uint64_t first_in(uint64_t a, uint64_t b) const {
    if (b <= pc->P) return kNone;
    const uint64_t pos = a < pc->P ? pc->P : a;
    for (uint64_t r = pc_region_of(*pc, pos - pc->P); r < pc->nregions; ++r) {
      const uint64_t base = pc->P + pc_region_base(*pc, r);
      if (base >= b) break;
      const uint32_t cnt = pc->region_cnt[r];
      const uint32_t n = cnt < pc->region_cap ? cnt : pc->region_cap;
      const uint32_t* l = pc->region_list + r * (uint64_t)pc->region_cap;
      const uint64_t ar = a > base ? a - base : 0;
      uint32_t lo = 0, hi = n;
      while (lo < hi) {
        const uint32_t m = (lo + hi) >> 1;
        if ((uint64_t)l[m] <= ar) lo = m + 1; else hi = m;
      }
      if (lo < n) {
        const uint64_t p = base + l[lo];
        return p <= b ? p : kNone;
      }
    }
    return kNone;
  }
};

template <class Src>
__device__ __forceinline__ uint64_t next_cut(uint64_t s, Src& src, const ChainParams& w) {
  uint64_t lim;
  if (w.is_last) {
    if (w.L - s <= w.min) return w.L;
    lim = s + w.max < w.L ? s + w.max : w.L;
  } else {
    lim = s + w.max;
  }
  const uint64_t c = src.first_in(s + w.min, lim);
  if (c != kNone) return c;
  if (!w.is_last && lim > w.PE) return kUndet;
  return lim;
}

constexpr uint32_t kWalkMaxRegions = 4096;

template <int NT>
__device__ uint32_t walk_block_scan(uint32_t v, uint32_t* s_wave, uint32_t* total) {
  const uint32_t lane = threadIdx.x & 63, wv = threadIdx.x >> 6;
  uint32_t incl = v;
#pragma unroll
  for (int d = 1; d < 64; d <<= 1) {
    const uint32_t t = __shfl_up(incl, d, 64);
    if (lane >= (uint32_t)d) incl += t;
  }
  if (lane == 63) s_wave[wv] = incl;
  __syncthreads();
  uint32_t before = 0, all = 0;
#pragma unroll
  for (int i = 0; i < NT / 64; ++i) {
    const uint32_t t = s_wave[i];
    before += (i < (int)wv) ? t : 0u;
    all += t;
  }
  __syncthreads();
  *total = all;
  return before + incl - v;
}

template <int NT>
__global__ __launch_bounds__(NT) void walk_kernel(StitchArgs a) {
  constexpr int kWalkThreads = NT;
  extern __shared__ __attribute__((aligned(16))) uint32_t smem[];
  uint32_t* cand = smem;
  uint64_t* xs = (uint64_t*)(smem + a.lds_cap);
  __shared__ uint32_t s_off[kWalkMaxRegions + 1];
  __shared__ uint32_t s_wave[kWalkThreads / 64];
  constexpr uint32_t kSpecLds = 4096;
  __shared__ uint32_t s_spec[kSpecLds];
  __shared__ uint32_t s_spec_n[kMaxSpg + 1];
  __shared__ uint32_t s_spec_end[kMaxSpg + 1];

  uint64_t* tr = (a.trace && threadIdx.x == 0) ? a.trace + 10ull * blockIdx.x : nullptr;
  if (tr) tr[0] = __builtin_amdgcn_s_memrealtime();
  DevState* st = a.state;
  const bool init = a.init != 0;
  const uint32_t done0 = init ? 0u : st->done;
  if (blockIdx.x == 0 && threadIdx.x == 0) {
    if (init) {
      st->carry = a.init_carry;
      st->total = 0;
      st->piece_cuts = 0;
      st->repaired = 0;
      st->discarded = 0;
      st->done = 0;
      st->err = 0;
      st->active = 0;
    }
    st->base = init ? 0ull : st->total;
    st->skip = (done0 || *a.pc.overflow) ? 1u : 0u;
  }
  if (done0 || *a.pc.overflow) return;
  const uint64_t s0 = init ? a.init_carry : uniform64(st->carry);
  const uint32_t kA = blockIdx.x * a.spg;
  if (kA >= a.nseg) return;
  const uint32_t kB = (kA + a.spg < a.nseg ? kA + a.spg : a.nseg) - 1;
  const uint32_t kFirst = kA > 0 ? kA - 1 : 0;
  const uint64_t lo = seg_start(a, s0, kFirst);
  const uint64_t hi = seg_end(a, kB);
  const PieceCands& pc = a.pc;

  const uint64_t r0 = lo <= pc.P ? 0 : pc_region_of(pc, lo - pc.P);
  uint64_t r1 = hi <= pc.P ? 0 : pc_region_of(pc, hi - pc.P - 1) + 1;
  if (r1 > pc.nregions) r1 = pc.nregions;
  const uint32_t nreg = r1 > r0 ? (uint32_t)(r1 - r0) : 0u;
  bool dense = nreg > kWalkMaxRegions;
  uint32_t total = 0;
  if (!dense) {
    for (uint32_t b = 0; b < nreg; b += kWalkThreads) {
      const uint32_t i = b + threadIdx.x;
      uint32_t c = 0;
      if (i < nreg) {
        c = pc.region_cnt[r0 + i];
        c = c < pc.region_cap ? c : pc.region_cap;
      }
      uint32_t part;
      const uint32_t ex = walk_block_scan<NT>(c, s_wave, &part);
      if (i < nreg) s_off[i] = total + ex;
      total += part;
    }
    if (threadIdx.x == 0) s_off[nreg] = total;
    __syncthreads();
    dense = total > a.lds_cap;
  }
  if (tr) tr[1] = __builtin_amdgcn_s_memrealtime();
  if (!dense) {
    for (uint32_t g = threadIdx.x; g < total; g += kWalkThreads) {
      uint32_t l = 0, h = nreg;
      while (h - l > 1) {
        const uint32_t m = (l + h) >> 1;
        if (s_off[m] <= g) l = m; else h = m;
      }
      const uint64_t r = r0 + l;
      const uint64_t p = pc.P + pc_region_base(pc, r) +
                         pc.region_list[r * (uint64_t)pc.region_cap + (g - s_off[l])];
      cand[g] = p <= lo ? 0u : (p > hi ? 0xFFFFFFFFu : (uint32_t)(p - lo));
    }
  }
  __syncthreads();
  if (tr) {
    tr[2] = __builtin_amdgcn_s_memrealtime();
    tr[5] = __builtin_amdgcn_s_memtime();
  }

  const uint32_t nwalk = kB - kFirst + 1;
  const RelChain rc = rel_chain(a.chain, lo);
  const uint32_t stride = min(a.scap, kSpecLds / nwalk);
  const uint32_t wv = __builtin_amdgcn_readfirstlane(threadIdx.x >> 6), ln = threadIdx.x & 63;
  constexpr uint32_t kWaves = kWalkThreads / 64;
  if (!dense) {
    for (uint32_t t = wv; t < nwalk; t += kWaves) {
      const uint32_t k = kFirst + t;
      const uint64_t v = seg_start(a, s0, k);
      const uint64_t e = seg_end(a, k);
      WaveLdsSrc src{cand, total, 0, lo, ln, 0};
      src.seek(v);
      if (tr && t == wv) tr[7] = __builtin_amdgcn_s_memrealtime();
      const uint32_t er = rel_clamp(e, lo);
      uint32_t x = rel_clamp(v, lo);
      uint32_t ns = 0, why = 0;
      uint32_t* spec_t = s_spec + t * stride;
      const uint32_t cap = __builtin_amdgcn_readfirstlane(rc.tail_at ? min(min(rc.lim_cap, er), rc.tail_at - 1u) : 0u);
      uint64_t cm = 0;
      auto flush = [&]() __attribute__((always_inline)) {
        if (cm) {
          const uint32_t idx = ns + __builtin_amdgcn_mbcnt_hi((uint32_t)(cm >> 32),
                                                             __builtin_amdgcn_mbcnt_lo((uint32_t)cm, 0u));
          if (((cm >> ln) & 1u) && idx < stride) spec_t[idx] = src.v;
          ns += (uint32_t)__builtin_popcountll(cm);
          cm = 0;
        }
      };
      while (true) {
        if (x < rc.tail_at) {
          uint64_t m = __ballot(src.v > x + rc.min);
          uint32_t l, c, lim, xm;
          asm volatile(
              "L_walk_step_%=:\n\t"
              "s_cmp_eq_u64 %[m], 0\n\t"
              "s_cbranch_scc1 L_walk_out_%=\n\t"
              "s_ff1_i32_b64 %[l], %[m]\n\t"
              "s_add_u32 %[lim], %[x], %[mx]\n\t"
              "v_readlane_b32 %[c], %[v], %[l]\n\t"
              "s_min_u32 %[lim], %[lim], %[cap]\n\t"
              "s_cmp_gt_u32 %[c], %[lim]\n\t"
              "s_cbranch_scc1 L_walk_out_%=\n\t"
              "s_bitset1_b64 %[cm], %[l]\n\t"
              "s_add_u32 %[xm], %[c], %[mn]\n\t"
              "s_mov_b32 %[x], %[c]\n\t"
              "v_cmp_lt_u32_e64 %[m], %[xm], %[v]\n\t"
              "s_branch L_walk_step_%=\n"
              "L_walk_out_%=:"
              : [m] "+s"(m), [x] "+s"(x), [cm] "+s"(cm), [l] "=&s"(l), [c] "=&s"(c),
                [lim] "=&s"(lim), [xm] "=&s"(xm)
              : [v] "v"(src.v), [mx] "s"(rc.max), [mn] "s"(rc.min), [cap] "s"(cap)
              : "scc");
        }
        flush();
        uint32_t nx;
        if (__builtin_expect(x >= rc.tail_at, 0)) {
          if (x >= rc.end_at) { why = 1; break; }
          nx = rc.L;
        } else {
          nx = rel_step(x, src, rc);
        }
        if (__builtin_expect(nx > er, 0)) {
          if (nx == kRelUndet) why = 2;
          break;
        }
        if (ln == 0 && ns < stride) spec_t[ns] = nx;
        ++ns;
        x = nx;
      }
      if (tr && t == wv) tr[9] = __builtin_amdgcn_s_memrealtime();
      const bool keep = ns <= stride;
      if (ln == 0) {
        xs[t] = lo + x;
        s_spec_n[t] = keep ? ns : 0xFFFFFFFFu;
        s_spec_end[t] = why;
        if (k >= kA) a.seg_info[k].X = lo + x;
      }
    }
  }
  __syncthreads();
  if (tr) {
    tr[3] = __builtin_amdgcn_s_memrealtime();
    uint32_t xcc, hwid;
    asm volatile("s_getreg_b32 %0, hwreg(HW_REG_XCC_ID, 0, 4)" : "=s"(xcc));
    asm volatile("s_getreg_b32 %0, hwreg(HW_REG_HW_ID)" : "=s"(hwid));
    tr[6] = ((uint64_t)xcc << 32) | hwid;
  }

  for (uint32_t i = wv; i < kB - kA + 1; i += kWaves) {
    const uint32_t k = kA + i;
    const uint32_t t = i + (kA - kFirst);
    SegInfo& si = a.seg_info[k];
    if (dense) {
      if (ln == 0) {
        si.E = kUndet;
        si.Z = kUndet;
        si.X = kUndet;
        si.cnt = 0;
        si.flags = kSegDense;
      }
      continue;
    }
    const uint64_t E = (k == 0) ? s0 : uniform64(xs[t - 1]);
    const uint64_t sst = seg_start(a, s0, k);
    const uint64_t e = seg_end(a, k);
    WaveLdsSrc src{cand, total, 0, lo, ln, 0};
    src.seek(E);
    uint64_t* out = a.stage + (uint64_t)k * a.scap;
    uint32_t n = 0, flags = 0;
    const uint32_t er = rel_clamp(e, lo), sr = rel_clamp(sst, lo);
    uint32_t x = rel_clamp(E, lo), last = x;
    const uint32_t sn = s_spec_n[t];
    const bool have_spec = sn != 0xFFFFFFFFu;
    const uint32_t* spec = s_spec + t * stride;
    const uint32_t specv = have_spec && ln < sn ? spec[ln] : 0xFFFFFFFFu;
    while (true) {
      uint32_t nx;
      if (__builtin_expect(x >= rc.tail_at, 0)) {
        if (x >= rc.end_at) { flags |= kSegEnd; break; }
        nx = rc.L;
      } else {
        nx = rel_step(x, src, rc);
      }
      if (__builtin_expect(nx > er, 0)) {
        if (nx == kRelUndet) flags |= kSegUndet;
        break;
      }
      if (nx > sr) {
        if (ln == (n & 63u) && n < a.scap) out[n] = lo + nx;
        ++n;
      }
      last = nx;
      x = nx;
      if (have_spec) {
        const uint64_t hit = __ballot(specv == nx);
        if (hit) {
          const uint32_t f = (uint32_t)__builtin_ctzll(hit);
          const uint32_t rest = sn - f - 1;
          for (uint32_t j = f + 1u + ln; j < sn; j += 64u)
            if (n + (j - f - 1u) < a.scap) out[n + (j - f - 1u)] = lo + spec[j];
          n += rest;
          if (rest) last = spec[sn - 1u];
          if (s_spec_end[t] == 1) flags |= kSegEnd;
          if (s_spec_end[t] == 2) flags |= kSegUndet;
          break;
        }
      }
    }
    if (n > a.scap) flags |= kSegOverflow;
    if (ln == 0) {
      si.E = E;
      si.Z = lo + last;
      si.cnt = n;
      si.flags = flags;
    }
  }
  if (a.trace) {
    __syncthreads();
    if (tr) tr[4] = __builtin_amdgcn_s_memrealtime();
  }
}

template __global__ void walk_kernel<256>(StitchArgs);
template __global__ void walk_kernel<1024>(StitchArgs);
template __global__ void walk_kernel<576>(StitchArgs);

constexpr int kFixThreads = 1024;

__device__ void publish(const StitchArgs& a, const DevState* st) {
  if (!a.host_state) return;
  publish_state(a.host_state, st, a.seq);
}

__global__ void publish_kernel(StitchArgs a) {
  if (threadIdx.x == 0 && blockIdx.x == 0) publish(a, a.state);
}

__global__ void noop_kernel() {}

__device__ uint32_t bsearch_u64(const uint64_t* v, uint32_t n, uint64_t x) {
  uint32_t l = 0, h = n;
  while (l < h) {
    const uint32_t m = (l + h) >> 1;
    if (v[m] < x) l = m + 1; else h = m;
  }
  return l;
}

template <int NT>
__device__ void fixup_body(const StitchArgs& a, bool do_publish = true) {
  __shared__ uint32_t s_flag_cnt;
  __shared__ uint64_t s_part[NT / 64];
  __shared__ int s_last_seg;
  __shared__ uint64_t s_carry, s_total0;
  DevState* st = a.state;
  if (threadIdx.x == 0) s_total0 = st->total;
  if (st->done || *a.pc.overflow) {
    if (threadIdx.x == 0) {
      st->active = 0;
      st->piece_cuts = 0;
      if (*a.pc.overflow) st->err |= kErrDense;
      if (do_publish) publish(a, st);
    }
    return;
  }
  const uint32_t T = a.nseg;
  const uint32_t kBad = kSegDense | kSegOverflow;

  if (threadIdx.x == 0) s_flag_cnt = 0;
  __syncthreads();
  for (uint32_t k = threadIdx.x; k < T; k += NT) {
    const SegInfo& si = a.seg_info[k];
    bool bad = (si.flags & kBad) != 0;
    if (k > 0) {
      const SegInfo& sp = a.seg_info[k - 1];
      bad = bad || (sp.X != sp.Z) || (sp.flags & kBad);
    }
    a.rep_cnt[k] = 0;
    a.rep_from[k] = 0;
    if (bad) a.flag_list[atomicAdd(&s_flag_cnt, 1u)] = k;
  }
  __syncthreads();
  const uint32_t nflag = s_flag_cnt;

  if (nflag > 0 && threadIdx.x == 0) {
    for (uint32_t i = 1; i < nflag; ++i) {
      const uint32_t v = a.flag_list[i];
      uint32_t j = i;
      while (j > 0 && a.flag_list[j - 1] > v) { a.flag_list[j] = a.flag_list[j - 1]; --j; }
      a.flag_list[j] = v;
    }
    GlobalSrc src{&a.pc};
    const uint64_t s0 = st->carry;
    uint32_t fi = 0, repaired = 0;
    uint64_t discarded = 0;
    uint32_t k = a.flag_list[0];
    bool rp = false;
    uint64_t rex = 0;
    while (k < T) {
      const SegInfo& si = a.seg_info[k];
      const uint64_t te = (k == 0) ? s0 : (rp ? rex : a.seg_info[k - 1].Z);
      if ((si.flags & kBad) == 0 && si.E == te) {
        rp = false;
        while (fi < nflag && a.flag_list[fi] <= k) ++fi;
        if (fi >= nflag) break;
        k = a.flag_list[fi];
        continue;
      }
      const uint64_t sst = (k == 0) ? s0 : a.anchor + (uint64_t)k * a.seg;
      const uint64_t e = seg_end(a, k);
      const uint64_t* stg = a.stage + (uint64_t)k * a.scap;
      const uint32_t scnt = (si.flags & kBad) ? 0u : si.cnt;
      uint64_t* rep = a.rep + (uint64_t)k * a.scap;
      uint32_t n = 0;
      uint64_t x = te, last = te;
      bool joined = false;
      while (true) {
        if (a.chain.is_last && x >= a.chain.L) break;
        const uint64_t nx = next_cut(x, src, a.chain);
        if (nx == kUndet || nx > e) break;
        if (nx > sst) {
          const uint32_t idx = bsearch_u64(stg, scnt, nx);
          if (idx < scnt && stg[idx] == nx) {
            joined = true;
            a.rep_from[k] = idx;
            break;
          }
          if (n < a.scap) rep[n] = nx;
          ++n;
        }
        last = nx;
        x = nx;
      }
      if (n > a.scap) st->err |= kErrCapacity;
      a.rep_cnt[k] = n;
      if (!joined) a.rep_from[k] = scnt;
      discarded += a.rep_from[k];
      ++repaired;
      rp = true;
      rex = joined ? si.Z : last;
      ++k;
    }
    st->repaired += repaired;
    st->discarded += discarded;
  }
  __syncthreads();

  const uint32_t per = (T + NT - 1) / NT;
  const uint32_t k0 = threadIdx.x * per < T ? threadIdx.x * per : T;
  const uint32_t k1 = (k0 + per < T) ? k0 + per : T;
  uint64_t mine = 0;
  int last_nonempty = -1;
  uint64_t my_last = 0;
  for (uint32_t k = k0; k < k1; ++k) {
    const SegInfo& si = a.seg_info[k];
    const uint32_t scnt = (si.flags & kBad) ? 0u : si.cnt;
    const uint32_t rc = a.rep_cnt[k], rf = a.rep_from[k];
    const uint64_t c = (uint64_t)rc + (scnt - rf);
    mine += c;
    if (c > 0) {
      last_nonempty = (int)k;
      my_last = scnt > rf ? a.stage[(uint64_t)k * a.scap + scnt - 1]
                          : a.rep[(uint64_t)k * a.scap + rc - 1];
    }
  }
  if (threadIdx.x == 0) s_last_seg = -1;
  const uint32_t lane = threadIdx.x & 63, wv = threadIdx.x >> 6;
  uint64_t incl = mine;
#pragma unroll
  for (int d = 1; d < 64; d <<= 1) {
    const uint64_t v = __shfl_up(incl, d, 64);
    if (lane >= (uint32_t)d) incl += v;
  }
  if (lane == 63) s_part[wv] = incl;
  __syncthreads();
  atomicMax(&s_last_seg, last_nonempty);
  if (threadIdx.x == 0) {
    uint64_t acc = 0;
    for (int i = 0; i < NT / 64; ++i) {
      const uint64_t v = s_part[i];
      s_part[i] = acc;
      acc += v;
    }
    st->piece_cuts = acc;
  }
  __syncthreads();
  uint64_t off = s_total0 + s_part[wv] + (incl - mine);
  for (uint32_t k = k0; k < k1; ++k) {
    const SegInfo& si = a.seg_info[k];
    const uint32_t scnt = (si.flags & kBad) ? 0u : si.cnt;
    a.out_off[k] = off;
    off += (uint64_t)a.rep_cnt[k] + (scnt - a.rep_from[k]);
  }
  if (last_nonempty >= 0 && last_nonempty == s_last_seg) s_carry = my_last;
  __syncthreads();
  if (threadIdx.x == 0) {
    const int ls = s_last_seg;
    if (ls >= 0) st->carry = s_carry;
    if (a.chain.is_last && st->carry >= a.chain.L) st->done = 1;
    const uint64_t tot = s_total0 + st->piece_cuts;
    if (tot > a.out_cap) st->err |= kErrCapacity;
    st->total = tot;
    st->active = 1;
    if (do_publish) publish(a, st);
  }
}

__global__ __launch_bounds__(kFixThreads) void fixup_kernel(StitchArgs a) {
  fixup_body<kFixThreads>(a, false);
}

template <int PER>
__global__ __launch_bounds__(kFixThreads) void fixup_fast_kernel(StitchArgs a) {
  constexpr int NT = kFixThreads;
  constexpr uint32_t kBad = kSegDense | kSegOverflow;
  __shared__ uint64_t s_lx[NT], s_lz[NT];
  __shared__ uint32_t s_lf[NT];
  __shared__ uint64_t s_part[NT / 64];
  __shared__ int s_last_seg;
  __shared__ uint64_t s_carry, s_piece;
  DevState* st = a.state;
  const uint32_t T = a.nseg;
  const uint32_t tid = threadIdx.x;
  const uint32_t k0 = tid * PER;
  const uint64_t total0 = st->total;
  const uint32_t done = st->done, ovf = *a.pc.overflow;
  uint64_t X[PER], Z[PER];
  uint32_t cnt[PER], fl[PER];
#pragma unroll
  for (int j = 0; j < PER; ++j) {
    X[j] = Z[j] = 0;
    cnt[j] = 0;
    fl[j] = 0;
    if (k0 + j < T) {
      const SegInfo& si = a.seg_info[k0 + j];
      X[j] = si.X;
      Z[j] = si.Z;
      cnt[j] = si.cnt;
      fl[j] = si.flags;
    }
  }
  if (done || ovf) {
    if (tid == 0) {
      st->active = 0;
      st->piece_cuts = 0;
      if (ovf) st->err |= kErrDense;
    }
    return;
  }
  s_lx[tid] = X[PER - 1];
  s_lz[tid] = Z[PER - 1];
  s_lf[tid] = fl[PER - 1];
  if (tid == 0) s_last_seg = -1;
  __syncthreads();
  bool bad = false;
#pragma unroll
  for (int j = 0; j < PER; ++j) {
    const uint32_t k = k0 + j;
    if (k >= T) break;
    bad = bad || (fl[j] & kBad) != 0;
    if (k > 0) {
      const uint64_t px = j ? X[j - 1] : s_lx[tid - 1];
      const uint64_t pz = j ? Z[j - 1] : s_lz[tid - 1];
      const uint32_t pf = j ? fl[j - 1] : s_lf[tid - 1];
      bad = bad || px != pz || (pf & kBad) != 0;
    }
  }
  if (__syncthreads_count(bad) != 0) {
    fixup_body<NT>(a, false);
    return;
  }
  uint64_t mine = 0, my_last = 0;
  int last_nonempty = -1;
#pragma unroll
  for (int j = 0; j < PER; ++j) {
    mine += cnt[j];
    if (cnt[j]) {
      last_nonempty = (int)(k0 + j);
      my_last = Z[j];
    }
  }
  const uint32_t lane = tid & 63, wv = tid >> 6;
  uint64_t incl = mine;
#pragma unroll
  for (int d = 1; d < 64; d <<= 1) {
    const uint64_t v = __shfl_up(incl, d, 64);
    if (lane >= (uint32_t)d) incl += v;
  }
  if (lane == 63) s_part[wv] = incl;
  atomicMax(&s_last_seg, last_nonempty);
  __syncthreads();
  if (tid == 0) {
    uint64_t acc = 0;
    for (int i = 0; i < NT / 64; ++i) {
      const uint64_t v = s_part[i];
      s_part[i] = acc;
      acc += v;
    }
    s_piece = acc;
  }
  __syncthreads();
  if (last_nonempty >= 0 && last_nonempty == s_last_seg) s_carry = my_last;
  const uint64_t piece = s_piece;
  const bool fits = total0 + piece <= a.out_cap;
  {
    uint64_t off = total0 + s_part[wv] + (incl - mine);
#pragma unroll
    for (int j = 0; j < PER; ++j) {
      if (k0 + j < T) {
        a.out_off[k0 + j] = off;
        a.rep_cnt[k0 + j] = 0;
        a.rep_from[k0 + j] = 0;
      }
      off += cnt[j];
    }
  }
  __syncthreads();
  if (tid == 0) {
    if (s_last_seg >= 0) st->carry = s_carry;
    if (a.chain.is_last && st->carry >= a.chain.L) st->done = 1;
    st->piece_cuts = piece;
    if (!fits) st->err |= kErrCapacity;
    st->total = total0 + piece;
    st->active = 1;
  }
}
template __global__ void fixup_fast_kernel<1>(StitchArgs);
template __global__ void fixup_fast_kernel<2>(StitchArgs);
template __global__ void fixup_fast_kernel<4>(StitchArgs);
template __global__ void fixup_fast_kernel<5>(StitchArgs);
template __global__ void fixup_fast_kernel<8>(StitchArgs);
template __global__ void fixup_fast_kernel<9>(StitchArgs);

constexpr int kFinThreads = 256;
constexpr uint32_t kFinMaxSeg = 2048;
constexpr uint32_t kFinSegPerWg = 16;

template <int PER>
__global__ __launch_bounds__(kFinThreads) void finish_kernel(StitchArgs a) {
  constexpr int NT = kFinThreads;
  constexpr uint32_t kBad = kSegDense | kSegOverflow;
  __shared__ uint64_t s_lx[NT], s_lz[NT];
  __shared__ uint32_t s_lf[NT];
  __shared__ uint64_t s_off[kFinMaxSeg];
  __shared__ uint32_t s_cnt[kFinMaxSeg];
  __shared__ uint64_t s_part[NT / 64];
  __shared__ int s_last_seg;
  __shared__ uint64_t s_carry, s_piece;
  DevState* st = a.state;
  const uint32_t T = a.nseg;
  const uint32_t tid = threadIdx.x;
  const uint32_t k0 = tid * PER;
  const uint32_t skip = st->skip;
  const uint64_t base = st->base;
  uint64_t X[PER], Z[PER];
  uint32_t cnt[PER], fl[PER];
#pragma unroll
  for (int j = 0; j < PER; ++j) {
    X[j] = Z[j] = 0;
    cnt[j] = 0;
    fl[j] = 0;
    if (k0 + j < T) {
      const SegInfo& si = a.seg_info[k0 + j];
      X[j] = si.X;
      Z[j] = si.Z;
      cnt[j] = si.cnt;
      fl[j] = si.flags;
    }
  }
  constexpr int QW = (int)kFinSegPerWg / (NT / 64);
  const uint32_t lane = tid & 63, wv = tid >> 6;
  const uint32_t kb = blockIdx.x * kFinSegPerWg;
  const uint32_t ke = kb + kFinSegPerWg < T ? kb + kFinSegPerWg : T;
  uint64_t v[QW];
  {
    const uint32_t sc1 = a.scap - 1;
#pragma unroll
    for (int q = 0; q < QW; ++q) {
      uint32_t k = kb + wv + (uint32_t)q * (NT / 64);
      k = k < T ? k : T - 1;
      v[q] = a.stage[(uint64_t)k * a.scap + (lane < sc1 ? lane : sc1)];
    }
  }
  const bool last_wg = blockIdx.x == gridDim.x - 1;
  if (skip) {
    if (last_wg && tid == 0) {
      st->active = 0;
      st->piece_cuts = 0;
      if (*a.pc.overflow) st->err |= kErrDense;
    }
    return;
  }
  s_lx[tid] = X[PER - 1];
  s_lz[tid] = Z[PER - 1];
  s_lf[tid] = fl[PER - 1];
  if (tid == 0) s_last_seg = -1;
  __syncthreads();
  bool bad = false;
#pragma unroll
  for (int j = 0; j < PER; ++j) {
    const uint32_t k = k0 + j;
    if (k >= T) break;
    bad = bad || (fl[j] & kBad) != 0;
    if (k > 0) {
      const uint64_t px = j ? X[j - 1] : s_lx[tid - 1];
      const uint64_t pz = j ? Z[j - 1] : s_lz[tid - 1];
      const uint32_t pf = j ? fl[j - 1] : s_lf[tid - 1];
      bad = bad || px != pz || (pf & kBad) != 0;
    }
  }
  if (__syncthreads_or(bad)) {
    if (blockIdx.x == 0) {
      fixup_body<NT>(a, false);
      __threadfence_block();
      __syncthreads();
      if (st->active && !(st->err & kErrCapacity)) {
        for (uint32_t k = tid; k < T; k += NT) {
          const uint32_t scnt = (a.seg_info[k].flags & kBad) ? 0u : a.seg_info[k].cnt;
          const uint32_t rc = a.rep_cnt[k], rf = a.rep_from[k];
          const uint64_t off = a.out_off[k];
          const uint64_t* rep = a.rep + (uint64_t)k * a.scap;
          const uint64_t* stg = a.stage + (uint64_t)k * a.scap;
          for (uint32_t i = 0; i < rc; ++i) a.out[off + i] = rep[i];
          for (uint32_t i = rf; i < scnt; ++i) a.out[off + rc + (i - rf)] = stg[i];
        }
      }
    }
    return;
  }
  uint64_t mine = 0, my_last = 0;
  int last_nonempty = -1;
#pragma unroll
  for (int j = 0; j < PER; ++j) {
    mine += cnt[j];
    if (cnt[j]) {
      last_nonempty = (int)(k0 + j);
      my_last = Z[j];
    }
  }
  uint64_t incl = mine;
#pragma unroll
  for (int d = 1; d < 64; d <<= 1) {
    const uint64_t v = __shfl_up(incl, d, 64);
    if (lane >= (uint32_t)d) incl += v;
  }
  if (lane == 63) s_part[wv] = incl;
  atomicMax(&s_last_seg, last_nonempty);
  __syncthreads();
  if (tid == 0) {
    uint64_t acc = 0;
    for (int i = 0; i < NT / 64; ++i) {
      const uint64_t v = s_part[i];
      s_part[i] = acc;
      acc += v;
    }
    s_piece = acc;
  }
  __syncthreads();
  {
    uint64_t off = base + s_part[wv] + (incl - mine);
#pragma unroll
    for (int j = 0; j < PER; ++j) {
      if (k0 + j < T) {
        s_off[k0 + j] = off;
        s_cnt[k0 + j] = cnt[j];
      }
      off += cnt[j];
    }
  }
  if (last_nonempty >= 0 && last_nonempty == s_last_seg) s_carry = my_last;
  __syncthreads();
  const uint64_t piece = s_piece;
  const bool fits = base + piece <= a.out_cap;
  if (fits) {
#pragma unroll
    for (int q = 0; q < QW; ++q) {
      const uint32_t k = kb + wv + (uint32_t)q * (NT / 64);
      if (k < ke && lane < s_cnt[k]) a.out[s_off[k] + lane] = v[q];
    }
#pragma unroll 1
    for (int q = 0; q < QW; ++q) {
      const uint32_t k = kb + wv + (uint32_t)q * (NT / 64);
      if (k >= ke) break;
      for (uint32_t i = 64 + lane; i < s_cnt[k]; i += 64)
        a.out[s_off[k] + i] = a.stage[(uint64_t)k * a.scap + i];
    }
  }
  if (last_wg && tid == 0) {
    if (s_last_seg >= 0) st->carry = s_carry;
    if (a.chain.is_last && st->carry >= a.chain.L) st->done = 1;
    st->piece_cuts = piece;
    if (!fits) st->err |= kErrCapacity;
    st->total = base + piece;
    st->active = 1;
  }
}
template __global__ void finish_kernel<1>(StitchArgs);
template __global__ void finish_kernel<2>(StitchArgs);
template __global__ void finish_kernel<4>(StitchArgs);
template __global__ void finish_kernel<8>(StitchArgs);

#if DSX_DIAG
__global__ __launch_bounds__(256) void stitch_task_kernel(TaskArgs b) {
  __shared__ __attribute__((aligned(16))) uint32_t cand[4 * kTaskCand];
  const uint32_t wave = __builtin_amdgcn_readfirstlane(threadIdx.x >> 6);
  const uint32_t lane = threadIdx.x & 63;
  const uint32_t t = blockIdx.x * 4u + wave;
  if (t < b.nf) finish_task(b.f, t, b.fseg, b.nf, b.farrive, lane);
  else if (t - b.nf < b.nw) walk_task(b.w, t - b.nf, b.wseg, cand + wave * kTaskCand, lane);
}
#endif

__global__ void state_init_kernel(DevState* st, uint64_t carry) {
  if (threadIdx.x == 0 && blockIdx.x == 0) {
    st->carry = carry;
    st->total = 0;
    st->piece_cuts = 0;
    st->repaired = 0;
    st->discarded = 0;
    st->done = 0;
    st->err = 0;
    st->active = 0;
  }
}

__global__ __launch_bounds__(256) void gather_kernel(StitchArgs a) {
  const uint32_t k = blockIdx.x;
  if (k >= a.nseg) return;
  if (!a.state->active || (a.state->err & kErrCapacity)) return;
  const SegInfo& si = a.seg_info[k];
  const uint32_t scnt = (si.flags & (kSegDense | kSegOverflow)) ? 0u : si.cnt;
  const uint32_t rc = a.rep_cnt[k], rf = a.rep_from[k];
  const uint64_t off = a.out_off[k];
  const uint64_t* rep = a.rep + (uint64_t)k * a.scap;
  const uint64_t* stg = a.stage + (uint64_t)k * a.scap;
  for (uint32_t i = threadIdx.x; i < rc; i += blockDim.x) a.out[off + i] = rep[i];
  for (uint32_t i = rf + threadIdx.x; i < scnt; i += blockDim.x) a.out[off + rc + (i - rf)] = stg[i];
}

}

#include "../../include/dsx.h"

namespace dsx {

__global__ __launch_bounds__(64) void seam_cands_kernel(PieceCands pc, uint64_t lo, uint64_t wend,
                                                        dsx_seam_t* seam) {
  const uint32_t lane = threadIdx.x;
  constexpr uint32_t kMax = DSX_SEAM_MAX_CANDS;
  uint32_t n = 0;
  const uint64_t r0 = lo > pc.P ? pc_region_of(pc, lo - pc.P) : 0;
  for (uint64_t r = r0; r < pc.nregions && n <= kMax; ++r) {
    const uint64_t base = pc.P + pc_region_base(pc, r);
    if (base >= wend) break;
    const uint32_t cnt0 = pc.region_cnt[r];
    const uint32_t cnt = cnt0 < pc.region_cap ? cnt0 : pc.region_cap;
    const uint32_t* l = pc.region_list + r * (uint64_t)pc.region_cap;
    for (uint32_t i0 = 0; i0 < cnt && n <= kMax; i0 += 64) {
      const uint32_t i = i0 + lane;
      const uint64_t p = i < cnt ? base + l[i] : 0;
      const bool ok = i < cnt && p > lo && p <= wend;
      const uint64_t m = __ballot(ok);
      const uint32_t idx = n + (uint32_t)__popcll(m & ((1ull << lane) - 1ull));
      if (ok) {
        if (idx < kMax) seam->cands[idx] = p;
        else if (idx == kMax) seam->first_cand_beyond = p;
      }
      n += (uint32_t)__popcll(m);
    }
  }
  if (lane == 0) {
    seam->ncands = n < kMax ? n : kMax;
    if (n <= kMax) seam->first_cand_beyond = ~0ull;
  }
}

__global__ void seam_finalize_kernel(dsx_seam_t* seam, const uint64_t* cuts, const DevState* st,
                                     uint64_t shard_start, uint64_t shard_len, uint64_t total,
                                     uint64_t wend0, uint64_t entry, uint32_t flags) {
  if (threadIdx.x != 0 || blockIdx.x != 0) return;
  uint64_t wend = wend0;
  if (seam->first_cand_beyond != ~0ull) wend = seam->cands[DSX_SEAM_MAX_CANDS - 1];
  const uint64_t n = st->total;
  uint32_t nc = 0;
  for (uint64_t i = 0; i < n; ++i) {
    const uint64_t x = cuts[i];
    if (x > wend) break;
    if (nc == DSX_SEAM_MAX_CUTS) {
      wend = seam->cuts[nc - 1];
      break;
    }
    seam->cuts[nc++] = x;
  }
  uint32_t ncand = 0;
  while (ncand < seam->ncands && seam->cands[ncand] <= wend) ++ncand;
  seam->shard_start = shard_start;
  seam->shard_len = shard_len;
  seam->total = total;
  seam->exit_cut = st->carry;
  seam->window_end = wend;
  seam->entry = entry;
  seam->ncands = ncand;
  seam->ncuts = nc;
  seam->flags = flags | (st->err ? (uint32_t)DSX_SEAM_REDO : 0u);
  seam->pad = 0;
}

struct SeamSrc {
  const uint64_t* c;
  uint32_t n;
  uint32_t j;
  __device__ uint64_t first_in(uint64_t a, uint64_t b) {
    while (j < n && c[j] <= a) ++j;
    if (j < n && c[j] <= b) return c[j];
    return kNone;
  }
};

__global__ void seam_resolve_kernel(const dsx_seam_t* all, int nranks, int rank, uint64_t min,
                                    uint64_t max, uint64_t* ext, uint64_t* info) {
  if (threadIdx.x != 0 || blockIdx.x != 0) return;
  for (int r = 0; r < nranks; ++r) {
    if (all[r].flags & DSX_SEAM_ERROR) {
      info[0] = kSeamPeerFailed;
      info[1] = (uint64_t)r;
      info[2] = 0;
      return;
    }
  }
  for (int r = 0; r < nranks; ++r) {
    if (all[r].flags & DSX_SEAM_REDO) {
      info[0] = kSeamRedo;
      info[1] = (uint64_t)r;
      info[2] = 0;
      return;
    }
  }
  uint64_t mine_c = all[rank].shard_start, mine_n = 0;
  uint64_t entry = all[0].exit_cut;
  for (int r = 1; r < nranks; ++r) {
    const dsx_seam_t& s = all[r];
    uint64_t c = kNone;
    uint32_t n = 0;
    if (s.flags & DSX_SEAM_REWALKED) {
      if (entry == s.entry) c = 0;
    } else if (entry == s.shard_start || s.shard_len == 0) {
      c = s.shard_start;
    } else {
      ChainParams w;
      w.min = min;
      w.max = max;
      w.L = s.total;
      w.PE = s.window_end;
      w.is_last = s.window_end == s.total ? 1u : 0u;
      w.pad = 0;
      SeamSrc src{s.cands, s.ncands, 0};
      uint64_t x = entry;
      while (true) {
        if (w.is_last && x >= w.L) { c = x; break; }
        const uint64_t nx = next_cut(x, src, w);
        if (nx == kUndet) break;
        const uint32_t idx = bsearch_u64(s.cuts, s.ncuts, nx);
        if (idx < s.ncuts && s.cuts[idx] == nx) { c = nx; break; }
        if (r == rank && n < DSX_SEAM_MAX_CUTS) ext[n++] = nx;
        x = nx;
      }
    }
    if (c == kNone) {
      info[0] = (uint64_t)r + 1;
      info[1] = entry;
      info[2] = 0;
      return;
    }
    if (r == rank) {
      mine_c = c;
      mine_n = n;
    }
    entry = s.shard_len == 0 ? entry : s.exit_cut;
  }
  info[0] = 0;
  info[1] = mine_c;
  info[2] = mine_n;
}

__global__ __launch_bounds__(256) void shard_emit_kernel(const uint64_t* info, const uint64_t* ext,
                                                         const uint64_t* spec, const DevState* st,
                                                         uint64_t* out, uint64_t cap,
                                                         volatile uint64_t* res, int32_t* code) {
  const uint64_t status = info[0];
  if (status != 0) {
    if (blockIdx.x == 0 && threadIdx.x == 0) {
      res[0] = status;
      res[1] = 0;
      res[2] = info[1];
      if (code) *code = status == kSeamPeerFailed ? 2 : 1;
      __threadfence_system();
    }
    return;
  }
  const uint64_t nspec = st->total;
  const uint64_t cr = info[1], next = info[2];
  uint64_t lo = 0, hi = nspec;
  while (lo < hi) {
    const uint64_t m = (lo + hi) >> 1;
    if (spec[m] < cr) lo = m + 1; else hi = m;
  }
  const uint64_t n = next + (nspec - lo);
  if (n <= cap) {
    for (uint64_t i = (uint64_t)blockIdx.x * blockDim.x + threadIdx.x; i < n;
         i += (uint64_t)gridDim.x * blockDim.x)
      out[i] = i < next ? ext[i] : spec[lo + (i - next)];
  }
  if (blockIdx.x == 0 && threadIdx.x == 0) {
    res[0] = 0;
    res[1] = n;
    res[2] = 0;
    if (code) *code = n <= cap ? 0 : 2;
    __threadfence_system();
  }
}

}
```

Baseline: 4631 GiB/s.

## Stitch large pieces as speculative slices in one walk launch with per-slice fixups

Splits each device piece into fixed-size slices (default 8 GiB) whose walks run together in one kernel launch. Each non-first slice starts speculatively from its anchor, and its fixup checks that the speculated start matches the carried chain state, falling back to the slow path otherwise. An optional single-call scan mode (off by default) enlarges the piece size. The aim is to expose more parallelism in stitching and to cut per-piece launch and serialization overhead, at the cost of extra fixup launches and a risk of speculation misses.

```diff
diff --git a/desync_amd/_lib.py b/desync_amd/_lib.py
--- a/desync_amd/_lib.py
+++ b/desync_amd/_lib.py
@@ -144,7 +144,8 @@
             "DSX_STREAM_BATCH": None, "DSX_NOOP_BEFORE_SCAN": None, "DSX_WALK_WGS": "2",
             "DSX_WALK_NT": "576", "DSX_TAIL_LOG": None, "DSX_FEED_THREADS": None, "DSX_FEED_MULTI": None,
             "DSX_FEED_MID": None, "DSX_SIDE_PRIO": "1",
-            "DSX_FEED_CUT_END": None, "DSX_SHARE_NS": "45", "DSX_SHARE_PC": "1", "DSX_SHARE_SLACK": "0", "DSX_CTX_PRIO": "1", "DSX_FEED_EXTRA": None, "DSX_SHARE_MULTI": "1", "DSX_FINE_TAIL": "33554432", "DSX_FINE_DIV": "4"}
+            "DSX_FEED_CUT_END": None, "DSX_SHARE_NS": "45", "DSX_SHARE_PC": "1", "DSX_SHARE_SLACK": "0", "DSX_CTX_PRIO": "1", "DSX_FEED_EXTRA": None, "DSX_SHARE_MULTI": "1", "DSX_FINE_TAIL": "33554432", "DSX_FINE_DIV": "4",
+            "DSX_CALL_SCAN": "0", "DSX_STITCH_SLICE": "8589934592"}
 
 
 def lib():
diff --git a/desync_amd/csrc/dsx_api.cpp b/desync_amd/csrc/dsx_api.cpp
--- a/desync_amd/csrc/dsx_api.cpp
+++ b/desync_amd/csrc/dsx_api.cpp
@@ -180,6 +180,9 @@
   }
   if (const char* v = getenv("DSX_STITCH_CUS")) c->stitch_cus = std::max(0, std::min(c->ncu / 2, atoi(v)));
   if (const char* v = getenv("DSX_SCAN_MASK")) c->scan_mask = atoi(v) != 0;
+  if (const char* v = getenv("DSX_CALL_SCAN")) c->call_scan = atoi(v) != 0;
+  if (const char* v = getenv("DSX_STITCH_SLICE"))
+    c->stitch_slice = (uint64_t)std::max(1L << 20, std::min((long)kPieceMax, atol(v)));
 #endif
   {
     int least = 0, greatest = 0;
@@ -423,6 +426,36 @@
   return DSX_OK;
 }
 
+static uint32_t line_lane_bytes(const dsx_ctx* c, uint64_t span, uint64_t slots_total) {
+  const uint64_t lanes_min = slots_total * 64 * (uint64_t)c->regions_per_slot;
+  const uint64_t per_lane = (span + lanes_min - 1) / lanes_min;
+  const uint64_t rounds_needed = (per_lane + kLineLaneMax - 1) / kLineLaneMax;
+  const uint64_t s = (span + rounds_needed * lanes_min - 1) / (rounds_needed * lanes_min);
+  uint64_t m = (s + 3 * kLine - 1) / (3 * kLine);
+  const uint64_t mcap = c->lane_target / (3 * kLine);
+  if (m > mcap + mcap / 4 || rounds_needed > 1) m = std::min<uint64_t>(m, mcap);
+  m = std::max<uint64_t>(1, std::min<uint64_t>(m, kLineLaneMax / (3 * kLine)));
+  uint32_t S = (uint32_t)(3 * kLine * m);
+  if (c->lane_bytes_override && c->lane_bytes_override % (3 * kLine) == 0 &&
+      c->lane_bytes_override <= kLineLaneMax)
+    S = c->lane_bytes_override;
+  return S;
+}
+
+static void line_tail_split(const dsx_ctx* c, uint64_t span, uint64_t slots_total, uint32_t S,
+                            uint64_t* nregions, uint64_t* nbig, uint64_t* S2) {
+  if (c->tail_split <= 1) return;
+  const uint64_t region_bytes = 64ull * S;
+  const uint64_t m = S / (3 * kLine), m2 = std::max<uint64_t>(1, m / (uint64_t)c->tail_split);
+  const uint64_t tail = slots_total * region_bytes * (uint64_t)c->tail_mult;
+  if (m2 < m && span >= 3 * tail) {
+    const uint64_t rb2 = 64ull * 3 * kLine * m2;
+    *nbig = (span - tail) / region_bytes;
+    *nregions = *nbig + (span - *nbig * region_bytes + rb2 - 1) / rb2;
+    *S2 = 3 * kLine * m2;
+  }
+}
+
 int enqueue_piece(dsx_ctx* c, const CallCfg& cc, const uint8_t* d_piece, uint64_t halo,
                          uint64_t P, uint64_t len, bool is_last) {
   const dsx_params_t* p = cc.p;
@@ -442,18 +475,7 @@
     S = kDenseS;
     LS = S;
   } else if (line) {
-    const uint64_t lanes_min = slots_total * 64 * (uint64_t)c->regions_per_slot;
-    const uint64_t per_lane = (span + lanes_min - 1) / lanes_min;
-    const uint64_t rounds_needed = (per_lane + kLineLaneMax - 1) / kLineLaneMax;
-    const uint64_t s = (span + rounds_needed * lanes_min - 1) / (rounds_needed * lanes_min);
-    uint64_t m = (s + 3 * kLine - 1) / (3 * kLine);
-    const uint64_t mcap = c->lane_target / (3 * kLine);
-    if (m > mcap + mcap / 4 || rounds_needed > 1) m = std::min<uint64_t>(m, mcap);
-    m = std::max<uint64_t>(1, std::min<uint64_t>(m, kLineLaneMax / (3 * kLine)));
-    S = (uint32_t)(3 * kLine * m);
-    if (c->lane_bytes_override && c->lane_bytes_override % (3 * kLine) == 0 &&
-        c->lane_bytes_override <= kLineLaneMax)
-      S = c->lane_bytes_override;
+    S = line_lane_bytes(c, span, slots_total);
     LS = kLaneSlots;
   } else {
     const uint64_t lanes_min = slots_total * 64 * (uint64_t)c->regions_per_slot;
@@ -474,16 +496,7 @@
   const uint64_t region_bytes = 64ull * S;
   uint64_t nregions = len == 0 ? 0 : (span + region_bytes - 1) / region_bytes;
   uint64_t nbig = nregions, S2 = 0;
-  if (line && !cc.dense && !cc.behind && c->tail_split > 1 && len > 0) {
-    const uint64_t m = S / (3 * kLine), m2 = std::max<uint64_t>(1, m / (uint64_t)c->tail_split);
-    const uint64_t tail = slots_total * region_bytes * (uint64_t)c->tail_mult;
-    if (m2 < m && span >= 3 * tail) {
-      const uint64_t rb2 = 64ull * 3 * kLine * m2;
-      nbig = (span - tail) / region_bytes;
-      nregions = nbig + (span - nbig * region_bytes + rb2 - 1) / rb2;
-      S2 = 3 * kLine * m2;
-    }
-  }
+  if (line && !cc.dense && !cc.behind && len > 0) line_tail_split(c, span, slots_total, S, &nregions, &nbig, &S2);
   const uint64_t nlanes = nregions * 64;
   uint32_t rcap;
   if (cc.dense) {
@@ -573,6 +586,7 @@
   }
 #endif
   const uint64_t seq = ++c->piece_seq;
+  const uint64_t lq = ++c->scan_seq;
   const int par = (int)(seq & 1);
   hipStream_t ss = c->scan_stream;
 
@@ -597,10 +611,10 @@
   sa.lane_slot = c->lane_slot.p;
   sa.region_cnt = rcnt;
   sa.region_list = rlist;
-  sa.overflow = c->overflow.p + (seq % kQueueSlots);
-  sa.overflow_next = c->overflow.p + ((seq + 1) % kQueueSlots);
-  sa.queue = c->overflow.p + 32 + 256 * (seq % kQueueSlots);
-  sa.queue_next = c->overflow.p + 32 + 256 * ((seq + 1) % kQueueSlots);
+  sa.overflow = c->overflow.p + (lq % kQueueSlots);
+  sa.overflow_next = c->overflow.p + ((lq + 1) % kQueueSlots);
+  sa.queue = c->overflow.p + 32 + 256 * (lq % kQueueSlots);
+  sa.queue_next = c->overflow.p + 32 + 256 * ((lq + 1) % kQueueSlots);
   sa.wave_major = c->wave_major ? (cc.behind ? 2u : 1u) : 0u;
   sa.nt_loads = (uint32_t)c->scan_nt;
   if (c->pub_host) {
@@ -786,7 +800,7 @@
     return DSX_OK;
   }
 #endif
-  int rc = launch_stitch(c, cc, pc, P, len, is_last, seq, line && c->scan_trace);
+  int rc = stitch_piece(c, cc, pc, P, len, is_last, seq, line && c->scan_trace);
   if (rc) return rc;
   if (split) HIPCHK(c, hipEventRecord(c->ev_stitch[par], c->stream));
   if (c->timing) HIPCHK(c, hipEventRecord(c->pev[3 * pi + 2], c->stream));
@@ -820,10 +834,169 @@
   return DSX_OK;
 }
 
+static uint64_t walk_spg(const dsx_ctx* c, const dsx_params_t* p, const PieceCands& pc, uint64_t seg,
+                         uint64_t nseg) {
+  const uint64_t region_bytes = pc.RB;
+  const double exp_per_seg = (double)seg / (double)p->discriminator + 8.0;
+  uint64_t spg = std::max<uint64_t>(2, nseg / ((uint64_t)c->walk_wgs * (uint64_t)c->ncu));
+  const bool wide = c->scan_stream != c->stream;
+  if (wide)
+    spg = std::max<uint64_t>(spg, (nseg + 2ull * c->stitch_cus - 1) / (2ull * c->stitch_cus));
+  spg = std::min<uint64_t>(spg, (uint64_t)((double)kWalkLdsCap / (2.0 * exp_per_seg)) - 1);
+  const uint64_t rb_min = pc.RB2 ? std::min<uint64_t>(region_bytes, pc.RB2) : region_bytes;
+  const uint64_t max_spg_reg = rb_min ? (4000ull * rb_min) / seg : kMaxSpg;
+  spg = std::min<uint64_t>(spg, max_spg_reg > 2 ? max_spg_reg - 2 : 1);
+  return std::max<uint64_t>(1, std::min<uint64_t>(spg, kMaxSpg));
+}
+
+static int stitch_buffers(dsx_ctx* c, StitchArgs& ta, uint64_t nseg) {
+  HIPCHK(c, grow(c, c->seg_info, nseg));
+  HIPCHK(c, grow(c, c->stage, nseg * ta.scap));
+  HIPCHK(c, grow(c, c->rep, nseg * ta.scap));
+  HIPCHK(c, grow(c, c->rep_cnt, nseg));
+  HIPCHK(c, grow(c, c->rep_from, nseg));
+  HIPCHK(c, grow(c, c->flag_list, nseg));
+  HIPCHK(c, grow(c, c->out_off, nseg));
+  ta.seg_info = c->seg_info.p;
+  ta.stage = c->stage.p;
+  ta.rep = c->rep.p;
+  ta.rep_cnt = c->rep_cnt.p;
+  ta.rep_from = c->rep_from.p;
+  ta.flag_list = c->flag_list.p;
+  ta.out_off = c->out_off.p;
+  return DSX_OK;
+}
+
+static int launch_fixup(dsx_ctx* c, const StitchArgs& ta) {
+  const uint64_t nseg = ta.nseg;
+  if (c->fixup_fast && nseg <= 9 * 1024) {
+    if (nseg <= 1024) hipLaunchKernelGGL(fixup_fast_kernel<1>, dim3(1), dim3(1024), 0, c->stream, ta);
+    else if (nseg <= 2048) hipLaunchKernelGGL(fixup_fast_kernel<2>, dim3(1), dim3(1024), 0, c->stream, ta);
+    else if (nseg <= 4096) hipLaunchKernelGGL(fixup_fast_kernel<4>, dim3(1), dim3(1024), 0, c->stream, ta);
+    else if (nseg <= 5120) hipLaunchKernelGGL(fixup_fast_kernel<5>, dim3(1), dim3(1024), 0, c->stream, ta);
+    else if (nseg <= 8192) hipLaunchKernelGGL(fixup_fast_kernel<8>, dim3(1), dim3(1024), 0, c->stream, ta);
+    else hipLaunchKernelGGL(fixup_fast_kernel<9>, dim3(1), dim3(1024), 0, c->stream, ta);
+  } else {
+    hipLaunchKernelGGL(fixup_kernel, dim3(1), dim3(1024), 0, c->stream, ta);
+  }
+  HIPCHK(c, hipGetLastError());
+  return DSX_OK;
+}
+
+static int launch_stitch_slices(dsx_ctx* c, const CallCfg& cc, const PieceCands& pc, uint64_t P,
+                                uint64_t len, bool is_last, uint64_t seq, bool trace) {
+  const dsx_params_t* p = cc.p;
+  const uint64_t slice = c->stitch_slice;
+  StitchArgs ta{};
+  ta.chain.min = p->min;
+  ta.chain.max = p->max;
+  ta.chain.L = cc.L;
+  ta.chain.PE = P + len;
+  ta.chain.is_last = is_last ? 1u : 0u;
+  ta.pc = pc;
+  ta.anchor = (P > cc.origin + p->max) ? P - p->max : cc.origin;
+  ta.seg = stitch_seg(c, p, slice + p->max);
+  ta.slice = slice;
+  ta.P0 = P;
+  ta.nslice = (uint32_t)((len + slice - 1) / slice);
+  ta.slice_segs = (uint32_t)((slice + p->max + ta.seg - 1) / ta.seg);
+  ta.spg = (uint32_t)walk_spg(c, p, pc, ta.seg, ta.slice_segs);
+  ta.slice_wgs = (ta.slice_segs + ta.spg - 1) / ta.spg;
+  ta.lds_cap = kWalkLdsCap;
+  ta.scap = (uint32_t)(ta.seg / p->min + 3);
+  const uint64_t nseg = (uint64_t)ta.nslice * ta.slice_segs;
+  int rc = stitch_buffers(c, ta, nseg);
+  if (rc) return rc;
+  ta.out = cc.d_out;
+  ta.out_cap = cc.out_cap;
+  ta.state = c->state.p;
+  ta.host_state = c->h_cur;
+  ta.seq = seq;
+  ta.init = c->init_pending ? 1u : 0u;
+  ta.init_carry = c->init_carry;
+  c->init_pending = false;
+  c->last_finish = false;
+  const uint64_t walk_grid = (uint64_t)ta.nslice * ta.slice_wgs;
+  if (trace && walk_grid <= 65536) {
+    ta.trace = c->trace.p + c->trace_base + kScanTraceWords * c->trace_n;
+    c->trace_walk_n = walk_grid;
+  }
+  const size_t walk_lds = (size_t)kWalkLdsCap * 4 + (kMaxSpg + 1) * 8;
+  if (c->walk_nt == 576 && ta.spg == 8)
+    hipLaunchKernelGGL(walk_slices_kernel<576>, dim3((uint32_t)walk_grid), dim3(576), walk_lds, c->stream, ta);
+  else
+    hipLaunchKernelGGL(walk_slices_kernel<256>, dim3((uint32_t)walk_grid), dim3(256), walk_lds, c->stream, ta);
+  HIPCHK(c, hipGetLastError());
+  for (uint32_t i = 0; i < ta.nslice; ++i) {
+    rc = launch_fixup(c, stitch_slice(ta, i));
+    if (rc) return rc;
+  }
+  hipLaunchKernelGGL(gather_slices_kernel, dim3((uint32_t)((nseg + 3) / 4)), dim3(256), 0, c->stream, ta);
+  HIPCHK(c, hipGetLastError());
+  return launch_publish(c, ta);
+}
+
+static bool slices_ok(const dsx_ctx* c, const dsx_params_t* p) {
+  return c->stitch_slice >= 8 * p->max &&
+         c->stitch_slice >= 2 * stitch_seg(c, p, c->stitch_slice + p->max);
+}
+
+int stitch_piece(dsx_ctx* c, const CallCfg& cc, const PieceCands& pc, uint64_t P, uint64_t len,
+                 bool is_last, uint64_t seq, bool trace) {
+  if (cc.slices && len > c->stitch_slice && slices_ok(c, cc.p))
+    return launch_stitch_slices(c, cc, pc, P, len, is_last, seq, trace);
+  return launch_stitch(c, cc, pc, P, len, is_last, seq, trace);
+}
+
+uint64_t device_piece(const dsx_ctx* c, const CallCfg& cc, const uint8_t* d_blob) {
+  if (cc.dense) return kDensePiece;
+  const uint64_t delta = (uintptr_t)d_blob & (kLine - 1);
+  const bool one = c->call_scan && cc.slices && !cc.behind && c->scan_line && cc.origin >= delta &&
+                   c->scan_stream == c->stream && slices_ok(c, cc.p);
+  return one ? std::max(kCallMax, c->stitch_slice) : c->stitch_slice;
+}
+
+#if DSX_DIAG
+extern "C" int dsx_diag_call_geometry(int ncu, uint64_t len, const dsx_params_t* p, uint64_t slice,
+                                      uint64_t* out) {
+  if (ncu <= 0 || !len || !p || !out || slice < 8 * p->max) return DSX_E_INVAL;
+  dsx_ctx c;
+  c.ncu = ncu;
+  c.stitch_slice = slice;
+  c.call_scan = true;
+  CallCfg cc{p, len, 0, kRound, nullptr, 0, false};
+  cc.slices = true;
+  const uint64_t piece = device_piece(&c, cc, nullptr);
+  const uint64_t span = std::min(piece, len);
+  const uint64_t slots_total = (uint64_t)c.ncu * c.scanl_waves;
+  const uint32_t S = line_lane_bytes(&c, span, slots_total);
+  uint64_t nregions = (span + 64ull * S - 1) / (64ull * S), nbig = nregions, S2 = 0;
+  line_tail_split(&c, span, slots_total, S, &nregions, &nbig, &S2);
+  StitchArgs ta{};
+  ta.chain.max = p->max;
+  ta.chain.L = len;
+  ta.chain.PE = span;
+  ta.chain.is_last = span == len;
+  ta.seg = stitch_seg(&c, p, slice + p->max);
+  ta.slice = slice;
+  ta.nslice = (uint32_t)((span + slice - 1) / slice);
+  out[0] = (len + piece - 1) / piece;
+  out[1] = nregions;
+  out[2] = nbig;
+  out[3] = S;
+  out[4] = S2;
+  out[5] = ta.nslice;
+  out[6] = ta.seg;
+  out[7] = slice_geo(ta, 0).nseg;
+  out[8] = ta.nslice > 2 ? slice_geo(ta, 1).nseg : 0;
+  out[9] = slice_geo(ta, ta.nslice - 1).nseg;
+  return DSX_OK;
+}
+#endif
+
 int launch_stitch(dsx_ctx* c, const CallCfg& cc, const PieceCands& pc, uint64_t P, uint64_t len,
                   bool is_last, uint64_t seq, bool trace) {
   const dsx_params_t* p = cc.p;
-  const uint64_t region_bytes = pc.RB;
   StitchArgs ta{};
   ta.chain.min = p->min;
   ta.chain.max = p->max;
@@ -838,33 +1011,15 @@
   ta.anchor = anchor;
   ta.seg = seg;
   ta.nseg = (uint32_t)nseg;
-  const double exp_per_seg = (double)seg / (double)p->discriminator + 8.0;
-  uint64_t spg = std::max<uint64_t>(2, nseg / ((uint64_t)c->walk_wgs * (uint64_t)c->ncu));
   const bool wide = c->scan_stream != c->stream;
-  if (wide)
-    spg = std::max<uint64_t>(spg, (nseg + 2ull * c->stitch_cus - 1) / (2ull * c->stitch_cus));
-  spg = std::min<uint64_t>(spg, (uint64_t)((double)kWalkLdsCap / (2.0 * exp_per_seg)) - 1);
-  const uint64_t rb_min = pc.RB2 ? std::min<uint64_t>(region_bytes, pc.RB2) : region_bytes;
-  const uint64_t max_spg_reg = rb_min ? (4000ull * rb_min) / seg : kMaxSpg;
-  spg = std::min<uint64_t>(spg, max_spg_reg > 2 ? max_spg_reg - 2 : 1);
-  spg = std::max<uint64_t>(1, std::min<uint64_t>(spg, kMaxSpg));
+  const uint64_t spg = walk_spg(c, p, pc, seg, nseg);
   ta.spg = (uint32_t)spg;
   ta.lds_cap = kWalkLdsCap;
   ta.scap = (uint32_t)(seg / p->min + 3);
-  HIPCHK(c, grow(c, c->seg_info, nseg));
-  HIPCHK(c, grow(c, c->stage, nseg * ta.scap));
-  HIPCHK(c, grow(c, c->rep, nseg * ta.scap));
-  HIPCHK(c, grow(c, c->rep_cnt, nseg));
-  HIPCHK(c, grow(c, c->rep_from, nseg));
-  HIPCHK(c, grow(c, c->flag_list, nseg));
-  HIPCHK(c, grow(c, c->out_off, nseg));
-  ta.seg_info = c->seg_info.p;
-  ta.stage = c->stage.p;
-  ta.rep = c->rep.p;
-  ta.rep_cnt = c->rep_cnt.p;
-  ta.rep_from = c->rep_from.p;
-  ta.flag_list = c->flag_list.p;
-  ta.out_off = c->out_off.p;
+  {
+    const int rcb = stitch_buffers(c, ta, nseg);
+    if (rcb) return rcb;
+  }
   ta.out = cc.d_out;
   ta.out_cap = cc.out_cap;
   ta.state = c->state.p;
@@ -896,17 +1051,10 @@
     HIPCHK(c, hipGetLastError());
     return launch_publish(c, ta);
   }
-  if (c->fixup_fast && nseg <= 9 * 1024) {
-    if (nseg <= 1024) hipLaunchKernelGGL(fixup_fast_kernel<1>, dim3(1), dim3(1024), 0, c->stream, ta);
-    else if (nseg <= 2048) hipLaunchKernelGGL(fixup_fast_kernel<2>, dim3(1), dim3(1024), 0, c->stream, ta);
-    else if (nseg <= 4096) hipLaunchKernelGGL(fixup_fast_kernel<4>, dim3(1), dim3(1024), 0, c->stream, ta);
-    else if (nseg <= 5120) hipLaunchKernelGGL(fixup_fast_kernel<5>, dim3(1), dim3(1024), 0, c->stream, ta);
-    else if (nseg <= 8192) hipLaunchKernelGGL(fixup_fast_kernel<8>, dim3(1), dim3(1024), 0, c->stream, ta);
-    else hipLaunchKernelGGL(fixup_fast_kernel<9>, dim3(1), dim3(1024), 0, c->stream, ta);
-  } else {
-    hipLaunchKernelGGL(fixup_kernel, dim3(1), dim3(1024), 0, c->stream, ta);
-  }
-  HIPCHK(c, hipGetLastError());
+  {
+    const int rcf = launch_fixup(c, ta);
+    if (rcf) return rcf;
+  }
   hipLaunchKernelGGL(gather_kernel, dim3((uint32_t)nseg), dim3(256), 0, c->stream, ta);
   HIPCHK(c, hipGetLastError());
   return launch_publish(c, ta);
@@ -916,7 +1064,8 @@
   HIPCHK(c, hipSetDevice(c->device));
   int rc = reset_state(c, cc.origin);
   if (rc) return rc;
-  const uint64_t piece = cc.dense ? kDensePiece : kPieceMax;
+  cc.slices = true;
+  const uint64_t piece = device_piece(c, cc, d_blob);
   for (uint64_t off = 0; off < len; off += piece) {
     if (c->cancel.load()) return DSX_E_INTERRUPTED;
     const uint64_t n = std::min(piece, len - off);
@@ -936,6 +1085,12 @@
                                   hipFuncAttributeMaxDynamicSharedMemorySize,
                                   (int)(kWalkLdsCap * 4 + (kMaxSpg + 1) * 8)));
     HIPCHK(c, hipFuncSetAttribute((const void*)walk_kernel<1024>,
+                                  hipFuncAttributeMaxDynamicSharedMemorySize,
+                                  (int)(kWalkLdsCap * 4 + (kMaxSpg + 1) * 8)));
+    HIPCHK(c, hipFuncSetAttribute((const void*)walk_slices_kernel<256>,
+                                  hipFuncAttributeMaxDynamicSharedMemorySize,
+                                  (int)(kWalkLdsCap * 4 + (kMaxSpg + 1) * 8)));
+    HIPCHK(c, hipFuncSetAttribute((const void*)walk_slices_kernel<576>,
                                   hipFuncAttributeMaxDynamicSharedMemorySize,
                                   (int)(kWalkLdsCap * 4 + (kMaxSpg + 1) * 8)));
     done = true;
@@ -1376,6 +1531,7 @@
     const bool dense = attempt == 1 || (rewalk && sh.dense);
     CallCfg cc{p, sh.total, entry, kRound, c->out.p, need, dense};
     cc.halo0 = sh.start > 0 ? sh.halo : 0;
+    cc.slices = true;
     int rc = DSX_OK;
     if (stitch_only) {
       HIPCHK(c, c->zero_word.ensure(1));
@@ -1387,8 +1543,8 @@
       for (size_t i = 0; i < sh.nkept && !rc; ++i) {
         PieceCands pc = sh.kept[i].pc;
         pc.overflow = c->zero_word.p;
-        rc = launch_stitch(c, cc, pc, sh.kept[i].P, sh.kept[i].len,
-                           is_last && i + 1 == sh.nkept, ++c->piece_seq, false);
+        rc = stitch_piece(c, cc, pc, sh.kept[i].P, sh.kept[i].len,
+                          is_last && i + 1 == sh.nkept, ++c->piece_seq, false);
       }
       if (rc) return rc;
       hipLaunchKernelGGL(seam_cands_kernel, dim3(1), dim3(64), 0, c->stream, sh.kept[0].pc,
@@ -1400,7 +1556,7 @@
       sh.dense = dense;
       rc = reset_state(c, entry);
       if (rc) return rc;
-      const uint64_t piece = cc.dense ? kDensePiece : kPieceMax;
+      const uint64_t piece = device_piece(c, cc, sh.d);
       for (uint64_t off = 0; off < sh.len; off += piece) {
         const uint64_t n = std::min(piece, sh.len - off);
         rc = enqueue_piece(c, cc, sh.d + off, off + cc.halo0, sh.start + off, n,
diff --git a/desync_amd/csrc/dsx_engine.h b/desync_amd/csrc/dsx_engine.h
--- a/desync_amd/csrc/dsx_engine.h
+++ b/desync_amd/csrc/dsx_engine.h
@@ -25,6 +25,9 @@
 __global__ void stitch_task_kernel(TaskArgs b);
 template <int NT>
 __global__ void walk_kernel(StitchArgs a);
+template <int NT>
+__global__ void walk_slices_kernel(StitchArgs a);
+__global__ void gather_slices_kernel(StitchArgs a);
 __global__ void fixup_kernel(StitchArgs a);
 template <int PER>
 __global__ void fixup_fast_kernel(StitchArgs a);
@@ -56,6 +59,7 @@
 namespace dsx_host {
 
 constexpr uint64_t kPieceMax = 8ull << 30;
+constexpr uint64_t kCallMax = 64ull << 30;
 constexpr uint64_t kStreamBatch = 16ull << 20;
 constexpr uint32_t kQueueDepth = 8;
 constexpr uint32_t kWalkLdsCap = 8192;
@@ -131,6 +135,8 @@
   int scan_nt = 1;
   bool finish = true;
   bool fixup_fast = true;
+  bool call_scan = false;
+  uint64_t stitch_slice = kPieceMax;
   DevBuf<uint64_t> trace;
   uint64_t trace_n = 0, trace_walk_n = 0;
   bool trace_keep = false;
@@ -154,6 +160,7 @@
   DevBuf<DevState> state;
   HostState* h_state = nullptr;
   uint64_t piece_seq = 0;
+  uint64_t scan_seq = 0;
   bool init_pending = false;
   uint64_t last_region_bytes = 0;
   uint32_t last_nregions = 0, last_region_cap = 0;
@@ -324,6 +331,7 @@
   uint64_t halo0 = 0;
   std::vector<KeptPiece>* keep = nullptr;
   bool behind = false;
+  bool slices = false;
 };
 
 int reset_state(dsx_ctx* c, uint64_t carry);
@@ -349,6 +357,9 @@
   } while (0)
 int launch_stitch(dsx_ctx* c, const CallCfg& cc, const PieceCands& pc, uint64_t P, uint64_t len,
                   bool is_last, uint64_t seq, bool trace);
+int stitch_piece(dsx_ctx* c, const CallCfg& cc, const PieceCands& pc, uint64_t P, uint64_t len,
+                 bool is_last, uint64_t seq, bool trace);
+uint64_t device_piece(const dsx_ctx* c, const CallCfg& cc, const uint8_t* d_blob);
 int launch_digest(dsx_ctx* c, DigestArgs da, uint64_t max_n, int algo, hipStream_t stream = nullptr,
                   uint32_t* queue = nullptr, bool serial = false, uint32_t max_blocks = 0, int pc = -1);
 void index_release(dsx_ctx* c);
diff --git a/desync_amd/csrc/dsx_stitch.h b/desync_amd/csrc/dsx_stitch.h
--- a/desync_amd/csrc/dsx_stitch.h
+++ b/desync_amd/csrc/dsx_stitch.h
@@ -132,7 +132,52 @@
   uint64_t* trace;
   uint64_t init_carry;
   uint32_t init;
-  uint32_t pad_init;
+  uint32_t spec0;
+  uint64_t slice;
+  uint64_t P0;
+  uint32_t nslice;
+  uint32_t slice_segs;
+  uint32_t slice_wgs;
+  uint32_t pad_slice;
+  uint64_t prev_start;
 };
 
+struct SliceGeo {
+  uint64_t PE, anchor;
+  uint32_t is_last, nseg;
+};
+__host__ __device__ __forceinline__ SliceGeo slice_geo(const StitchArgs& a, uint32_t i) {
+  SliceGeo g;
+  const uint64_t P = a.P0 + (uint64_t)i * a.slice;
+  const bool last = i + 1 >= a.nslice;
+  g.PE = last ? a.chain.PE : P + a.slice;
+  g.is_last = last ? a.chain.is_last : 0u;
+  g.anchor = i > 0 ? P - a.chain.max : a.anchor;
+  const uint64_t end = g.is_last ? a.chain.L : g.PE;
+  g.nseg = end > g.anchor ? (uint32_t)((end - g.anchor + a.seg - 1) / a.seg) : 1u;
+  return g;
 }
+__host__ __device__ __forceinline__ StitchArgs stitch_slice(const StitchArgs& a, uint32_t i) {
+  StitchArgs s = a;
+  const SliceGeo g = slice_geo(a, i);
+  s.chain.PE = g.PE;
+  s.chain.is_last = g.is_last;
+  s.anchor = g.anchor;
+  s.nseg = g.nseg;
+  if (i > 0) {
+    s.spec0 = 1u;
+    s.prev_start = g.anchor + a.chain.max - a.seg;
+  }
+  const uint64_t k0 = (uint64_t)i * a.slice_segs;
+  s.seg_info += k0;
+  s.stage += k0 * a.scap;
+  s.rep += k0 * a.scap;
+  s.rep_cnt += k0;
+  s.rep_from += k0;
+  s.flag_list += k0;
+  s.out_off += k0;
+  s.nslice = 0;
+  return s;
+}
+
+}
diff --git a/desync_amd/csrc/dsx_stitch.hip b/desync_amd/csrc/dsx_stitch.hip
--- a/desync_amd/csrc/dsx_stitch.hip
+++ b/desync_amd/csrc/dsx_stitch.hip
@@ -101,7 +101,7 @@
 }
 
 template <int NT>
-__global__ __launch_bounds__(NT) void walk_kernel(StitchArgs a) {
+__device__ __forceinline__ void walk_body(const StitchArgs& a, const uint32_t bx) {
   constexpr int kWalkThreads = NT;
   extern __shared__ __attribute__((aligned(16))) uint32_t smem[];
   uint32_t* cand = smem;
@@ -118,7 +118,7 @@
   DevState* st = a.state;
   const bool init = a.init != 0;
   const uint32_t done0 = init ? 0u : st->done;
-  if (blockIdx.x == 0 && threadIdx.x == 0) {
+  if (bx == 0 && threadIdx.x == 0 && !a.spec0) {
     if (init) {
       st->carry = a.init_carry;
       st->total = 0;
@@ -133,12 +133,13 @@
     st->skip = (done0 || *a.pc.overflow) ? 1u : 0u;
   }
   if (done0 || *a.pc.overflow) return;
-  const uint64_t s0 = init ? a.init_carry : uniform64(st->carry);
-  const uint32_t kA = blockIdx.x * a.spg;
+  const uint64_t s0 = a.spec0 ? a.anchor : init ? a.init_carry : uniform64(st->carry);
+  const uint32_t kA = bx * a.spg;
   if (kA >= a.nseg) return;
   const uint32_t kB = (kA + a.spg < a.nseg ? kA + a.spg : a.nseg) - 1;
   const uint32_t kFirst = kA > 0 ? kA - 1 : 0;
-  const uint64_t lo = seg_start(a, s0, kFirst);
+  const uint32_t pre = (a.spec0 && bx == 0) ? 1u : 0u;
+  const uint64_t lo = pre ? a.prev_start : seg_start(a, s0, kFirst);
   const uint64_t hi = seg_end(a, kB);
   const PieceCands& pc = a.pc;
 
@@ -185,16 +186,17 @@
     tr[5] = __builtin_amdgcn_s_memtime();
   }
 
-  const uint32_t nwalk = kB - kFirst + 1;
+  const uint32_t nwalk = kB - kFirst + 1 + pre;
   const RelChain rc = rel_chain(a.chain, lo);
   const uint32_t stride = min(a.scap, kSpecLds / nwalk);
   const uint32_t wv = __builtin_amdgcn_readfirstlane(threadIdx.x >> 6), ln = threadIdx.x & 63;
   constexpr uint32_t kWaves = kWalkThreads / 64;
   if (!dense) {
     for (uint32_t t = wv; t < nwalk; t += kWaves) {
-      const uint32_t k = kFirst + t;
-      const uint64_t v = seg_start(a, s0, k);
-      const uint64_t e = seg_end(a, k);
+      const bool isprev = pre && t == 0;
+      const uint32_t k = kFirst + t - pre;
+      const uint64_t v = isprev ? a.prev_start : seg_start(a, s0, k);
+      const uint64_t e = isprev ? a.anchor + a.chain.max : seg_end(a, k);
       WaveLdsSrc src{cand, total, 0, lo, ln, 0};
       src.seek(v);
       if (tr && t == wv) tr[7] = __builtin_amdgcn_s_memrealtime();
@@ -260,7 +262,7 @@
         xs[t] = lo + x;
         s_spec_n[t] = keep ? ns : 0xFFFFFFFFu;
         s_spec_end[t] = why;
-        if (k >= kA) a.seg_info[k].X = lo + x;
+        if (!isprev && k >= kA) a.seg_info[k].X = lo + x;
       }
     }
   }
@@ -275,7 +277,7 @@
 
   for (uint32_t i = wv; i < kB - kA + 1; i += kWaves) {
     const uint32_t k = kA + i;
-    const uint32_t t = i + (kA - kFirst);
+    const uint32_t t = i + (kA - kFirst) + pre;
     SegInfo& si = a.seg_info[k];
     if (dense) {
       if (ln == 0) {
@@ -287,7 +289,7 @@
       }
       continue;
     }
-    const uint64_t E = (k == 0) ? s0 : uniform64(xs[t - 1]);
+    const uint64_t E = (k == 0 && !pre) ? s0 : uniform64(xs[t - 1]);
     const uint64_t sst = seg_start(a, s0, k);
     const uint64_t e = seg_end(a, k);
     WaveLdsSrc src{cand, total, 0, lo, ln, 0};
@@ -347,6 +349,20 @@
   }
 }
 
+template <int NT>
+__global__ __launch_bounds__(NT) void walk_kernel(StitchArgs a) {
+  walk_body<NT>(a, blockIdx.x);
+}
+
+template <int NT>
+__global__ __launch_bounds__(NT) void walk_slices_kernel(StitchArgs a) {
+  const uint32_t i = blockIdx.x / a.slice_wgs;
+  const StitchArgs s = stitch_slice(a, i);
+  walk_body<NT>(s, blockIdx.x - i * a.slice_wgs);
+}
+template __global__ void walk_slices_kernel<256>(StitchArgs);
+template __global__ void walk_slices_kernel<576>(StitchArgs);
+
 template __global__ void walk_kernel<256>(StitchArgs);
 template __global__ void walk_kernel<1024>(StitchArgs);
 template __global__ void walk_kernel<576>(StitchArgs);
@@ -401,6 +417,8 @@
     if (k > 0) {
       const SegInfo& sp = a.seg_info[k - 1];
       bad = bad || (sp.X != sp.Z) || (sp.flags & kBad);
+    } else if (a.spec0) {
+      bad = bad || si.E != st->carry;
     }
     a.rep_cnt[k] = 0;
     a.rep_from[k] = 0;
@@ -551,6 +569,7 @@
   const uint32_t k0 = tid * PER;
   const uint64_t total0 = st->total;
   const uint32_t done = st->done, ovf = *a.pc.overflow;
+  const bool e0_bad = a.spec0 && tid == 0 && a.seg_info[0].E != st->carry;
   uint64_t X[PER], Z[PER];
   uint32_t cnt[PER], fl[PER];
 #pragma unroll
@@ -579,7 +598,7 @@
   s_lf[tid] = fl[PER - 1];
   if (tid == 0) s_last_seg = -1;
   __syncthreads();
-  bool bad = false;
+  bool bad = e0_bad;
 #pragma unroll
   for (int j = 0; j < PER; ++j) {
     const uint32_t k = k0 + j;
@@ -862,6 +881,22 @@
   const uint64_t* stg = a.stage + (uint64_t)k * a.scap;
   for (uint32_t i = threadIdx.x; i < rc; i += blockDim.x) a.out[off + i] = rep[i];
   for (uint32_t i = rf + threadIdx.x; i < scnt; i += blockDim.x) a.out[off + rc + (i - rf)] = stg[i];
+}
+__global__ __launch_bounds__(256) void gather_slices_kernel(StitchArgs a) {
+  const uint32_t w = blockIdx.x * 4u + __builtin_amdgcn_readfirstlane(threadIdx.x >> 6);
+  const uint32_t i = w / a.slice_segs, k = w - i * a.slice_segs;
+  if (i >= a.nslice || k >= slice_geo(a, i).nseg) return;
+  if (!a.state->active || (a.state->err & kErrCapacity)) return;
+  const uint64_t g = (uint64_t)i * a.slice_segs + k;
+  const SegInfo& si = a.seg_info[g];
+  const uint32_t scnt = (si.flags & (kSegDense | kSegOverflow)) ? 0u : si.cnt;
+  const uint32_t rc = a.rep_cnt[g], rf = a.rep_from[g];
+  const uint64_t off = a.out_off[g];
+  const uint64_t* rep = a.rep + g * a.scap;
+  const uint64_t* stg = a.stage + g * a.scap;
+  const uint32_t ln = threadIdx.x & 63u;
+  for (uint32_t j = ln; j < rc; j += 64u) a.out[off + j] = rep[j];
+  for (uint32_t j = rf + ln; j < scnt; j += 64u) a.out[off + rc + (j - rf)] = stg[j];
 }
 
 }
```

Result: no change. 4633 GiB/s (median of 2 runs) (+0.0%).
